# pengpeng-yu/FastPCC

Measured on AMD Instinct MI355X. Metric: encode+decode Mpoints/sec, lossy_coord_v2 baseline_r1 (stream of 16-frame batches, 2 in flight; one frame at a time = value_one_frame), higher is better.
Workload: dtype f32; 1 GPU; lossy_coord_v2/baseline_r1 inference, 997645-voxel 1024^3 body-surface frames (cfg#2), seeded random-init weights; one step = a batch of 16 such frames per GPU (15966320 voxels) through compress_many + decompress_many = ONE network traversal over the batch, 16 independent streams; 2 batch(es) in flight per GPU; parallelism=single GPU, 2 batches in flight per GPU on one stream (fastpcc_amd/serving.py), batch_clouds=16, frames_in_flight=2, named_stages=False, bytes=143901, coder_handover_retries=0

## Files before the change

fastpcc_amd/codecs/lossy_coord_v2/layers.py:

```python
from typing import List, Optional, Tuple

import torch
import torch.nn as nn
import torch.nn.functional as F

from ... import engine as ME
from ... import hipops as ops
from ...sparse_conv_layers import ConvBlock, ConvTransBlock, GenConvTransBlock, MEMLPBlock, \
    NNSequentialWithConvBlockArgs, NNSequentialWithConvTransBlockArgs, mlp_chain_forward


def _run(seq: nn.Sequential, x, last_clip: float = 0.0):
    mods = list(seq)
    for m in mods[:-1]:
        x = m(x)
    return mods[-1](x, clip=last_clip) if last_clip > 0 else mods[-1](x)


def classify_head(seq: nn.Sequential, fea):
    blocks = list(seq)
    ok = len(blocks) == 2 and not torch.is_grad_enabled() and len(fea.parts) == 1
    if ok:
        a, b = blocks
        ok = all(isinstance(m, ConvBlock) and m.bn is None and m.conv.ks == 1 and
                 (m.act_module is None or isinstance(m.act_module, (ME.MinkowskiPReLU, ME.MinkowskiReLU))) for m in blocks) and \
            b.conv.out_channels == 1 and a.conv.out_channels == b.conv.in_channels and \
            ops.pointwise_head_ok(a.conv.in_channels, a.conv.out_channels)
    x = fea.parts[0] if ok else None
    if not ok or x.dtype != torch.float32 or x.stride(1) != 1 or (x.shape[0] > 1 and x.stride(0) % 4) or x.data_ptr() % 16:
        return seq(fea)
    da, db = a.conv._derived(), b.conv._derived()
    act1, act2 = ME._act_of(a.act_module), ME._act_of(b.act_module)
    cm = fea.coordinate_manager
    orders = {ME.summation_order('k1', a.conv.in_channels, 0, a.conv.out_channels, rows)
              for rows in cm.cloud_rows(cm._map(fea.coordinate_map_key)) if rows > 0}
    if len(orders) != 1 or not orders <= {0, 1}:
        return seq(fea)
    order1 = orders.pop()
    out = ops.pointwise_head(x, da['w'].reshape(a.conv.in_channels, a.conv.out_channels), da['b'], act1.kind, act1.slope, order1,
                             db['w'].reshape(-1), db['b'], act2.kind, act2.slope)
    return ME.SparseTensor(out, coordinate_map_key=fea.coordinate_map_key, coordinate_manager=fea.coordinate_manager)


class Encoder(nn.Module):

    def __init__(self, in_channels: int, intra_channels: Tuple[int, ...], requires_points_num_list: bool,
                 points_num_scaler: float, region_type: str, act: Optional[str]):
        super().__init__()
        self.requires_points_num_list = requires_points_num_list
        self.points_num_scaler = points_num_scaler
        stages = [ConvBlock(in_channels, intra_channels[0], 3, 1, region_type=region_type, act=act)]
        for c_prev, c in zip(intra_channels[:-1], intra_channels[1:]):
            stages.append(nn.Sequential(
                ConvBlock(c_prev, c, 2, 2, region_type='HYPER_CUBE', act=act),
                ConvBlock(c, c, 3, 1, region_type=region_type, act=act)))
        self.blocks = nn.ModuleList(stages)

    def forward(self, x) -> Tuple[ME.SparseTensor, Optional[List[List[int]]]]:
        counts = []
        last = len(self.blocks) - 1
        for i, block in enumerate(self.blocks):
            x = block(x)
            if i != last:
                cm = x.coordinate_manager
                edges = cm.batch_offsets(cm._map(x.coordinate_map_key))
                counts.append([b - a for a, b in zip(edges[:-1], edges[1:])])
        if not self.requires_points_num_list:
            return x, None
        return x, [[int(n * self.points_num_scaler) for n in c] for c in counts]


class Decoder(nn.Module):

    def __init__(self, in_channels: int, intra_channels: Tuple[int, ...], region_type: str, act: Optional[str]):
        super().__init__()
        self.upsample_blocks = nn.ModuleList()
        self.classify_blocks = nn.ModuleList()
        prev = in_channels
        n_stage = len(intra_channels)
        for i, ch in enumerate(intra_channels):
            up = nn.Sequential()
            if i == n_stage - 1:
                up.append(ConvBlock(prev, prev, 3, 1, region_type=region_type, act=act))
            up.append(GenConvTransBlock(prev, ch, 2, 2, region_type='HYPER_CUBE', act=act))
            if i != n_stage - 1:
                up.append(ConvBlock(ch, ch, 3, 1, region_type=region_type, act=act))
            self.upsample_blocks.append(up)
            self.classify_blocks.append(nn.Sequential(ConvBlock(ch, ch // 2, 1, 1, act=act),
                                                      ConvBlock(ch // 2, 1, 1, 1, act=None)))
            prev = ch
        self.pruning = ME.MinkowskiPruning()

    def forward(self, fea, points_num_list, coord_offset=None):
        if self.training:
            return self.train_forward(fea, points_num_list, coord_offset)
        return self.test_forward(fea, points_num_list, coord_offset)

    def train_forward(self, fea, points_num_list, target_key: ME.CoordinateMapKey) -> dict:
        loss = {}
        n_stage = len(self.upsample_blocks)
        cm = fea.coordinate_manager
        top = cm._map(fea.coordinate_map_key)
        inv = [1 / sum(c) for c in points_num_list] if points_num_list is not None else None
        for i, (up, classify) in enumerate(zip(self.upsample_blocks, self.classify_blocks)):
            fea = up(fea)
            pred = classify(fea)
            keep = self.get_keep_train(pred, points_num_list, top)
            target = self.get_target(pred, target_key)
            keep |= target
            loss[f'coord_{n_stage - i - 1}_recon_loss'] = F.binary_cross_entropy_with_logits(
                pred.F.squeeze(1), target.to(pred.F.dtype), reduction='sum')
            if i != n_stage - 1:
                fea = self.pruning(fea, keep.to(torch.uint8))
        if inv is not None and len(inv) != 1:
            total = sum(inv)
            for i in range(n_stage):
                loss[f'coord_{i}_recon_loss'] = loss[f'coord_{i}_recon_loss'] * (inv[i] / total * len(inv))
        return loss

    @torch.no_grad()
    def get_target(self, pred: ME.SparseTensor, target_key: ME.CoordinateMapKey) -> torch.Tensor:
        cm = pred.coordinate_manager
        gen = cm._map(pred.coordinate_map_key)
        tgt = cm._map(cm.stride(target_key, pred.tensor_stride))
        if gen.generated and tgt.parent is gen.parent:
            self.last_target_path = 'child_table'
            return ops.child_mask(tgt.child_row).bool()
        if gen.level != tgt.level or gen.bits != tgt.bits:
            raise ValueError('candidates and strided target set differ in tensor stride')
        self.last_target_path = 'keys_member'
        return ops.keys_member(cm._keys(tgt), cm._keys(gen)) >= 0

    @torch.no_grad()
    def get_keep_train(self, pred: ME.SparseTensor, points_num_list: Optional[List[List[int]]], top) -> torch.Tensor:
        cm = pred.coordinate_manager
        gen = cm._map(pred.coordinate_map_key)
        if not gen.generated:
            raise NotImplementedError('get_keep expects the candidates of a generative upsampling')
        parent = gen.parent
        logits = pred.F.detach().reshape(-1).contiguous()
        cell = None
        if parent is not top:
            cell = cm._ancestor_rows(parent, top).to(torch.int32).contiguous()
        if points_num_list is None:
            return fixed_keep(logits, cell, 0 if cell is None else top.n).bool()
        targets = points_num_list.pop()
        edges = cm.batch_offsets(parent)
        if len(targets) != len(edges) - 1:
            raise ValueError('one pruning target per sample expected')
        return ops.topk_keep_batch(logits, edges, targets, cell, 0 if cell is None else top.n).bool()

    @torch.no_grad()
    def test_forward(self, fea, points_num_list, coord_offset: Optional[torch.Tensor] = None):
        last = len(self.upsample_blocks) - 1
        cm = fea.coordinate_manager
        top = cm._map(fea.coordinate_map_key)
        for i, (up, classify) in enumerate(zip(self.upsample_blocks, self.classify_blocks)):
            fea = up(fea)
            keep = self.get_keep(classify_head(classify, fea), points_num_list, top)
            if i != last:
                fea = self.pruning(fea, keep)
            else:
                gen = cm._map(fea.coordinate_map_key)
                if not gen.generated:
                    raise RuntimeError('decoder output is expected on a generated coordinate set')
                if not cm.independent_clouds:
                    xyz, count = ops.compact_coords(gen.parent.keys, keep, gen.level, gen.bits, coord_offset)
                    return xyz[:int(count.item())]
                edges = cm.batch_offsets(gen.parent)
                parts = [ops.compact_coords(gen.parent.keys[a:b], keep[8 * a: 8 * b], gen.level, gen.bits,
                                            None if coord_offset is None else coord_offset[c].contiguous())
                         for c, (a, b) in enumerate(zip(edges[:-1], edges[1:]))]
                counts = torch.cat([count for _, count in parts]).tolist()
                return [xyz[:n] for (xyz, _), n in zip(parts, counts)]

    @torch.no_grad()
    def get_keep(self, pred: ME.SparseTensor, points_num_list: Optional[List[List[int]]], top=None) -> torch.Tensor:
        cm = pred.coordinate_manager
        gen = cm._map(pred.coordinate_map_key)
        if not gen.generated:
            raise NotImplementedError('get_keep expects the candidates of a generative upsampling')
        logits = pred.F.view(-1)
        parent = gen.parent
        cell = None
        if top is not None and parent is not top:
            cell, m = parent.parent_of, parent.parent
            while m is not top:
                if m is None or m.parent_of is None:
                    raise RuntimeError('candidate set is not below the decoder input level')
                cell, m = m.parent_of[cell.long()], m.parent
            cell = cell.to(torch.int32).contiguous()
        if points_num_list is None:
            return fixed_keep(logits, cell, 0 if cell is None else top.n)
        return adaptive_keep(cm, parent, top, logits, cell, points_num_list.pop())


def fixed_keep(logits: torch.Tensor, cell: Optional[torch.Tensor], n_cells: int) -> torch.Tensor:
    groups = logits.view(-1, 8)
    per_group = groups.max(1).values
    if cell is None:
        return ((groups > 0) | (groups == per_group[:, None])).view(-1).to(torch.uint8)
    cell_max = torch.full((n_cells,), float('-inf'), dtype=per_group.dtype, device=per_group.device)
    cell_max.scatter_reduce_(0, cell.long(), per_group, reduce='amax', include_self=True)
    return ((groups > 0) | (groups == cell_max[cell.long()][:, None])).view(-1).to(torch.uint8)


def adaptive_keep(cm, parent, top, logits: torch.Tensor, cell: Optional[torch.Tensor], target: List[int]) -> torch.Tensor:
    if cm.independent_clouds:
        edges = cm.batch_offsets(parent)
        if len(target) != len(edges) - 1:
            raise ValueError('one pruning target per cloud expected')
        return ops.topk_keep_batch(logits, edges, target, cell, 0 if cell is None else top.n)
    if len(target) != 1:
        raise NotImplementedError('batch size 1 at test time, as in the reference (model.py:121)')
    if not logits.numel() > target[0]:
        raise ValueError('fewer candidates than points to keep')
    if cell is None:
        return ops.topk_keep(logits, target[0])
    return ops.topk_keep_cells(logits, cell, top.n, target[0])


class HyperDecoderUpsample(nn.Module):

    def __init__(self, in_channels: Tuple[int, ...], out_channels: Tuple[int, ...], if_sample: Tuple[int, ...],
                 region_type: str, act: Optional[str]):
        super().__init__()
        self.blocks = nn.ModuleList()
        for c_in, c_out, up in zip(in_channels, out_channels, if_sample):
            if up:
                head = ConvTransBlock(max(c_in, 1), c_out, 2, 2, region_type=region_type, act=act)
                seq = NNSequentialWithConvTransBlockArgs
            else:
                head = ConvBlock(max(c_in, 1), c_out, 3, 1, region_type=region_type, act=act)
                seq = NNSequentialWithConvBlockArgs
            self.blocks.append(seq(head, ConvBlock(c_out, c_out, 3, 1, region_type=region_type, act=act)))

    def __len__(self):
        return len(self.blocks)

    def __getitem__(self, idx):
        return self.blocks[idx]


class HyperDecoderGenUpsample(nn.Module):

    def __init__(self, in_channels: Tuple[int, ...], if_sample: Tuple[int, ...], region_type: str, act: Optional[str]):
        super().__init__()
        self.blocks = nn.ModuleList()
        for c_in, up in zip(in_channels, if_sample):
            if not up:
                self.blocks.append(None)
                continue
            mid = max(c_in // 4, 1)
            self.blocks.append(nn.Sequential(
                GenConvTransBlock(c_in, mid, 2, 2, region_type=region_type, act=act),
                ConvBlock(mid, 1, 3, 1, region_type=region_type, act=None)))

    def __getitem__(self, idx):
        return self.blocks[idx]


class SubResidualGeoLossl(nn.Module):

    def __init__(self, in_ch, out_ch, region_type, act, bottleneck_value_bound: int):
        super().__init__()
        self.blocks = nn.Sequential(
            ConvBlock(in_ch + in_ch, in_ch, 3, 1, region_type=region_type, act=act),
            ConvBlock(in_ch, out_ch, 3, 1, region_type=region_type, act=None))
        self.register_buffer('bound', torch.tensor(bottleneck_value_bound), persistent=False)
        self._bound = float(bottleneck_value_bound)

    def forward(self, x, y):
        return _run(self.blocks, ME.cat(x, y), last_clip=self._bound)


class ResidualGeoLossl(nn.Module):
    def __init__(self, in_channels: Tuple[int, ...], out_channels: Tuple[int, ...], region_type: str,
                 act: Optional[str], bottleneck_value_bound: int, skip_encoding_fea: int):
        super().__init__()
        self.blocks = nn.ModuleList()
        for idx, (c_in, c_out) in enumerate(zip(in_channels, out_channels)):
            self.blocks.append(SubResidualGeoLossl(c_in, c_out, region_type, act, bottleneck_value_bound)
                               if idx > skip_encoding_fea else None)

    def __len__(self):
        return len(self.blocks)

    def __getitem__(self, idx):
        return self.blocks[idx]


class SubDecoderGeoLossl(nn.Module):

    def __init__(self, in_ch, in_ch2, out_ch, region_type, act):
        super().__init__()
        self.residual_decoder = nn.Sequential(MEMLPBlock(in_ch, out_ch // 2, act=act),
                                              MEMLPBlock(out_ch // 2, out_ch, act=act))
        self.decoder = nn.Sequential(MEMLPBlock(out_ch + in_ch2, out_ch, act=act),
                                     MEMLPBlock(out_ch, out_ch, act=act))

    def forward(self, x, y: ME.SparseTensor):
        fused = mlp_chain_forward([*self.residual_decoder, *self.decoder], x, y, cat_layer=len(self.residual_decoder))
        if fused is not None:
            return ME.SparseTensor(fused, coordinate_map_key=y.coordinate_map_key, coordinate_manager=y.coordinate_manager)
        if isinstance(x, torch.Tensor):
            x = ME.SparseTensor(x, coordinate_map_key=y.coordinate_map_key, coordinate_manager=y.coordinate_manager)
        return self.decoder(ME.cat(self.residual_decoder(x), y))


class SubDecoderGeoLossl2(nn.Module):
    def __init__(self, in_ch, in_ch2, out_ch, region_type, act):
        super().__init__()
# ... 63 lines not shown
```

fastpcc_amd/csrc/hip/conv.hip:

```cpp
#include "conv_common.h"
#include <atomic>
#include <cstdlib>

namespace fpcc {
namespace {

template <int NBT, int CH, int WM, int WN>
struct MfmaCfg {
    static constexpr int C_OUT = 32 * NBT;
    static constexpr int TM = 32 * WM;
    static constexpr int NBW = NBT / WN;
    static constexpr int THREADS = 64 * WM * WN;
    static constexpr int G8 = CH / 8;
    static constexpr int W_TOTAL = CH * C_OUT / 4;
    static constexpr int W_PIECES = (W_TOTAL + THREADS - 1) / THREADS;
    static_assert(NBT % WN == 0, "column blocks must divide over the waves");
};

template <typename C, int CH>
__device__ __forceinline__ void fetch_a(const ConvArgs &a, const int32_t *nbr_rows, int cc, int li, int lh,
                                        f32x4 (&ra)[C::G8]) {
    const bool in_x1 = cc * CH < a.c1;
    const float *xb = in_x1 ? a.x1 + cc * CH : a.x2 + (cc * CH - a.c1);
    const int64_t ld = in_x1 ? a.ld1 : a.ld2;
// ... 813 lines not shown
        const float *ap[2], *bp;
        auto next_stage = [&]() {
            const bool in1 = cc_f < n1;
            const int c = in1 ? cc_f : cc_f - n1;
            ap[0] = (in1 ? a1[0] : a2[0]) + c * step[0];
            ap[1] = (in1 ? a1[1] : a2[1]) + c * step[1];
            bp = bpk + cc_f * chunk_floats;
            if (cc_f + 1 < n_chunks) {
                ++cc_f;
            } else {
                const unsigned r2 = rest & (rest - 1);
                if (r2) { rest = r2; cc_f = 0; set_offset(__ffs(r2) - 1); }
            }
        };
        f32x4 ra[2][G8], rbv[G8][2];
        next_stage();
#pragma unroll
        for (int g8 = 0; g8 < G8; ++g8) {
            __builtin_amdgcn_sched_barrier(0);
            ra[0][g8] = *reinterpret_cast<const f32x4 *>(ap[0] + 8 * g8);
            __builtin_amdgcn_sched_barrier(0);
            ra[1][g8] = *reinterpret_cast<const f32x4 *>(ap[1] + 8 * g8);
#pragma unroll
            for (int nb = 0; nb < 2; ++nb) {
                __builtin_amdgcn_sched_barrier(0);
                rbv[g8][nb] = *reinterpret_cast<const f32x4 *>(bp + ((int64_t)g8 * nbt + nb) * 256);
            }
        }
        __builtin_amdgcn_sched_barrier(0);
        for (int s = 0; s < n_stages; ++s) {
            if (cc_c == 0) {
                const int gk = offset_group_of(__ffs(rest_c) - 1, n_off);
                if (gk != cur_g) {
                    fold_acc();
                    for (int gz = cur_g + 1; gz < gk; ++gz) fold_zero();
                    cur_g = gk;
                }
            }
            if (++cc_c == n_chunks) { cc_c = 0; rest_c &= rest_c - 1; }
            next_stage();
            __builtin_amdgcn_sched_barrier(SB);
#pragma unroll
            for (int g8 = 0; g8 < G8; ++g8) {
                const f32x4 av0 = ra[0][g8], av1 = ra[1][g8];
                const f32x4 b0 = rbv[g8][0], b1 = rbv[g8][1];
#define FPCC_STEP(c)                                                                                     \
                acc[0][0] = __builtin_amdgcn_mfma_f32_32x32x2f32(av0.c, b0.c, acc[0][0], 0, 0, 0);       \
                acc[0][1] = __builtin_amdgcn_mfma_f32_32x32x2f32(av0.c, b1.c, acc[0][1], 0, 0, 0);       \
                acc[1][0] = __builtin_amdgcn_mfma_f32_32x32x2f32(av1.c, b0.c, acc[1][0], 0, 0, 0);       \
                acc[1][1] = __builtin_amdgcn_mfma_f32_32x32x2f32(av1.c, b1.c, acc[1][1], 0, 0, 0);
                FPCC_STEP(x) FPCC_STEP(y) FPCC_STEP(z) FPCC_STEP(w)
#undef FPCC_STEP
                __builtin_amdgcn_sched_barrier(SB);
                ra[0][g8] = *reinterpret_cast<const f32x4 *>(ap[0] + 8 * g8);
                __builtin_amdgcn_sched_barrier(SB);
                ra[1][g8] = *reinterpret_cast<const f32x4 *>(ap[1] + 8 * g8);
#pragma unroll
                for (int nb = 0; nb < 2; ++nb) {
                    __builtin_amdgcn_sched_barrier(SB);
                    rbv[g8][nb] = *reinterpret_cast<const f32x4 *>(bp + ((int64_t)g8 * nbt + nb) * 256);
                }
                __builtin_amdgcn_sched_barrier(SB);
            }
        }
    }
    if (wmask) { fold_acc(); ++cur_g; }
    for (int gz = cur_g; gz < 4; ++gz) fold_zero();

    const float slope = (a.act == FPCC_ACT_PRELU && a.slope) ? a.slope[0] : 0.0f;
    float bias2[2];
#pragma unroll
    for (int nb = 0; nb < 2; ++nb) bias2[nb] = a.bias ? a.bias[32 * ((int)cg * 2 + nb) + li] : 0.0f;
#pragma unroll
    for (int rb = 0; rb < 2; ++rb) {
        int64_t dsts[16];
#pragma unroll
        for (int reg = 0; reg < 16; ++reg) {
            const int64_t o = __shfl(my_row, 32 * rb + (reg & 3) + 8 * (reg >> 2) + 4 * lh);
            dsts[reg] = o < 0 ? -1 : o;
        }
#pragma unroll
        for (int reg = 0; reg < 16; ++reg) {
            const int64_t dst = dsts[reg];
            if (dst < 0) continue;
#pragma unroll
            for (int nb = 0; nb < 2; ++nb)
                a.out[dst * a.ldo + 32 * ((int)cg * 2 + nb) + li] = finish(tsum[rb][nb][reg], bias2[nb], a.act, slope, a.clip);
        }
    }
}

__global__ __launch_bounds__(256) void k_pack_weights(const float *__restrict__ w, int64_t n_mats, int c_in, int c_out,
                                                      float *__restrict__ wp) {
    const int64_t e = (int64_t)blockIdx.x * 256 + threadIdx.x;
    const int64_t per_mat = (int64_t)c_in * c_out;
    if (e >= n_mats * per_mat) return;
    const int nbt = c_out / 32;
    const int64_t m = e / per_mat;
    int64_t r = e - m * per_mat;
    const int j = (int)(r & 3); r >>= 2;
    const int i = (int)(r & 31); r >>= 5;
    const int h = (int)(r & 1); r >>= 1;
    const int nb = (int)(r % nbt); r /= nbt;
    const int g8 = (int)(r & 3); r >>= 2;
    const int cc = (int)r;
    wp[e] = w[m * per_mat + (int64_t)(32 * cc + 8 * g8 + 4 * h + j) * c_out + 32 * nb + i];
}

__global__ __launch_bounds__(256) void k_pack_weights_nat(const float *__restrict__ w, int64_t n_mats, int c_in, int c_out,
                                                          float *__restrict__ wp) {
    const int64_t e = (int64_t)blockIdx.x * 256 + threadIdx.x;
    const int64_t per_mat = (int64_t)c_in * c_out;
    if (e >= n_mats * per_mat) return;
    const int nbt = c_out / 32;
    const int64_t m = e / per_mat;
    int64_t r = e - m * per_mat;
    const int j = (int)(r & 3); r >>= 2;
    const int i = (int)(r & 31); r >>= 5;
    const int h = (int)(r & 1); r >>= 1;
    const int nb = (int)(r % nbt); r /= nbt;
    const int g8 = (int)(r & 3); r >>= 2;
    const int cc = (int)r;
    wp[e] = w[m * per_mat + (int64_t)(32 * cc + 8 * g8 + 2 * j + h) * c_out + 32 * nb + i];
}

inline bool aligned16(const void *p) { return (reinterpret_cast<uintptr_t>(p) & 15) == 0; }

int mfma_chunk(int c1, int c2, int c_out) {
    if (c_out != 32 && c_out != 64 && c_out != 128) return 0;
    const int c_in = c1 + c2;
    if (c_in % 32 == 0 && c1 % 32 == 0) return 32;
    if (c_in % 16 == 0 && c1 % 16 == 0) return 16;
    return 0;
}

bool natural_shape(int c1, int c2, int c_out, int n_offsets, int groups) {
    return c_out == 256 && c1 >= 32 && c1 % 32 == 0 && c2 >= 0 && c2 % 32 == 0 && c1 + c2 <= 512 && n_offsets >= 1 && n_offsets <= kMaxOffsets &&
           (groups == 1 || groups == 8);
}

int knob(int k);

template <int NBT, int CH, int WM, int WN>
int launch_mfma_cfg(ConvArgs a, hipStream_t s) {
    constexpr int TM = 32 * WM;
    const unsigned tiles = (unsigned)((a.n_out + TM - 1) / TM);
    const dim3 grid(tiles, a.groups), block(64 * WM * WN);
    hipLaunchKernelGGL((k_conv_mfma<NBT, CH, WM, WN>), grid, block, 0, s, a);
    return check_hip(hipGetLastError(), "k_conv_mfma");
}

enum { kKnobWaveOn = 0, kKnobWaveNbw = 1, kKnobWaveSb = 2, kKnobStamps = 3, kKnobGroupedFoldRows = 4, kKnobMfmaCfg = 5, kKnobPointwiseRows = 6,
       kKnobGroupedOff = 7, kKnobGroupedNbw = 8, kKnobWave22Rows = 9, kKnobLdsRows = 10, kKnobLdsRowBlocks = 11, kKnobPersist = 12, kKnobFold64 = 13, kKnobK2s2tSparse = 14,
       kKnobNaturalMfma = 15, kKnobCount = 16 };
int g_knob[kKnobCount] = {-1, -1, -1, -1, -1, -1, -1, -1, -1, -1, -1, -1, -1, -1, -1, -1};
int knob(int k) {
    if (g_knob[k] < 0) {
        static const char *names[kKnobCount] = {"FPCC_CONV_WAVE", "FPCC_WAVE_NBW", "FPCC_WAVE_SB", "", "FPCC_GROUPED_FOLD_ROWS",
                                                "FPCC_MFMA_TILE", "FPCC_POINTWISE_MIN_ROWS", "", "FPCC_GROUPED_NBW",
                                                "FPCC_WAVE22_MIN_ROWS", "FPCC_LDS_MIN_ROWS", "FPCC_LDS_ROW_BLOCKS",
                                                "FPCC_CONV_PERSIST", "FPCC_CONV_FOLD64", "FPCC_K2S2T_SPARSE",
                                                "FPCC_CONV_NATURAL_MFMA"};
        static const int defaults[kKnobCount] = {1, 0, 1, 0, 100 * 1024, 0, 32 * 1024, 0, 0, 0, 0, 2, 0, 0, 0, 2};
        const char *e = names[k][0] ? getenv(names[k]) : nullptr;
        g_knob[k] = e ? atoi(e) : defaults[k];
    }
    return g_knob[k];
}

template <int NBT, int CH>
int launch_mfma(const ConvArgs &a, hipStream_t s) {
    const int forced = knob(kKnobMfmaCfg) - 1;
    const int64_t work = a.n_out * a.groups;
    constexpr int WNS = NBT >= 2 ? 2 : 1;
    const int cfg = forced >= 0 ? forced : (NBT <= 2 && work >= 128 * 1024) ? 0 : work >= 32 * 1024 ? 1 : 2;
    if (cfg == 0) return launch_mfma_cfg<NBT, CH, 4, 1>(a, s);
    if (cfg == 1) return launch_mfma_cfg<NBT, CH, 2, WNS>(a, s);
    return launch_mfma_cfg<NBT, CH, 1, NBT>(a, s);
}

__global__ __launch_bounds__(256) void k_conv_c1_pointwise(ConvArgs a) {
    const int64_t e = (int64_t)blockIdx.x * 256 + threadIdx.x;
    if (e >= a.n_out * a.c_out) return;
    const int64_t o = e / a.c_out;
    const int j = (int)(e - o * a.c_out);
    const float slope = (a.act == FPCC_ACT_PRELU && a.slope) ? a.slope[0] : 0.0f;
    a.out[o * a.ldo + j] = finish(fmaf(a.x1[o * a.ld1], a.w[j], 0.0f), a.bias ? a.bias[j] : 0.0f, a.act, slope, a.clip);
}

template <int NBW>
int launch_wave_cfg(const ConvArgs &a, const float *wp, int nbt, hipStream_t s) {
    const int64_t row_blocks = (a.n_out + 31) / 32;
    const int64_t units = row_blocks * (nbt / NBW);
    if (units > 0x7fffffffll) return fail_arg("conv_f32: too many work units");
    const dim3 grid((unsigned)((units + 3) / 4), a.groups);
    if (knob(kKnobWaveSb)) hipLaunchKernelGGL((k_conv_wave<NBW, 32, 0x6>), grid, dim3(256), 0, s, a, wp, nbt, (unsigned)units);
    else hipLaunchKernelGGL((k_conv_wave<NBW, 32, 0>), grid, dim3(256), 0, s, a, wp, nbt, (unsigned)units);
    return check_hip(hipGetLastError(), "k_conv_wave");
}

constexpr int kMaxDevices = 16;
inline int current_device() {
    int dev = 0;
    return (hipGetDevice(&dev) == hipSuccess && dev >= 0 && dev < kMaxDevices) ? dev : -1;
}
int cu_count() {
    static std::atomic<int> cached[kMaxDevices];
    const int dev = current_device();
    if (dev < 0) return 256;
    int n = cached[dev].load(std::memory_order_relaxed);
    if (n == 0) {
        hipDeviceProp_t prop;
        n = (hipGetDeviceProperties(&prop, dev) == hipSuccess && prop.multiProcessorCount > 0) ? prop.multiProcessorCount : 256;
        cached[dev].store(n, std::memory_order_relaxed);
    }
    return n;
}

constexpr int kUnitCounters = 256;
__device__ unsigned g_unit_counters[kUnitCounters];
unsigned *next_unit_counter(unsigned start, hipStream_t s, int *rc) {
    static std::atomic<unsigned> seq{0};
    static std::atomic<unsigned *> bases[kMaxDevices];
    const int dev = current_device();
    if (dev < 0) {
        *rc = fail_arg("unit counters: no current device");
        return nullptr;
    }
    unsigned *base = bases[dev].load(std::memory_order_acquire);
    if (!base) {
        if (hipGetSymbolAddress(reinterpret_cast<void **>(&base), HIP_SYMBOL(g_unit_counters)) != hipSuccess) {
            *rc = check_hip(hipGetLastError(), "unit counters");
            return nullptr;
        }
        bases[dev].store(base, std::memory_order_release);
    }
    unsigned *c = base + (seq++ % kUnitCounters);
    *rc = check_hip(hipMemsetD32Async(reinterpret_cast<hipDeviceptr_t>(c), (int)start, 1, s), "unit counter fill");
    return c;
}

inline int64_t persist_slots() {
    const int v = knob(kKnobPersist);
    return v > 16 ? v : (int64_t)v * cu_count();
}
inline bool persist_ok(const ConvArgs &a) {
    return knob(kKnobPersist) > 0 && a.nbr && a.nbr_ks == 1 && (a.nbr_os & 3) == 0 && a.nbr_os >= ((a.n_off + 3) & ~3) &&
           (reinterpret_cast<uintptr_t>(a.nbr) & 15) == 0 && a.groups == 1;
}

template <int NBW>
int launch_grouped_cfg(const ConvArgs &a, const float *wp, int nbt, hipStream_t s) {
    const int64_t row_blocks = (a.n_out + 31) / 32;
    const int64_t units = row_blocks * (nbt / NBW);
    if (units > 0x7fffffffll) return fail_arg("conv_f32: too many work units");
    const bool stamps = knob(kKnobStamps) != 0;
    const int64_t slots = persist_slots();
    if (!stamps && persist_ok(a) && units > slots) {
        int rc = FPCC_OK;
        unsigned *counter = next_unit_counter((unsigned)slots, s, &rc);
        if (rc != FPCC_OK) return rc;
        hipLaunchKernelGGL((k_conv_wave<NBW, 32, 0x6, false, 4, false, true>), dim3((unsigned)slots, 1), dim3(256), 0, s, a, wp, nbt, (unsigned)units,
                           counter);
        return check_hip(hipGetLastError(), "k_conv_wave(grouped, persistent)");
    }
    if (stamps)
        hipLaunchKernelGGL((k_conv_wave<NBW, 32, 0x6, true, 4>), dim3((unsigned)units, a.groups), dim3(256), 0, s, a, wp, nbt, (unsigned)units);
    else
        hipLaunchKernelGGL((k_conv_wave<NBW, 32, 0x6, false, 4>), dim3((unsigned)units, a.groups), dim3(256), 0, s, a, wp, nbt, (unsigned)units);
    return check_hip(hipGetLastError(), "k_conv_wave(grouped)");
}

template <int NBW>
int launch_folded_cfg(const ConvArgs &a, const float *wp, int nbt, hipStream_t s) {
    const int64_t units = ((a.n_out + 31) / 32) * (nbt / NBW);
    if (units > 0x7fffffffll) return fail_arg("conv_f32: too many work units");
    const int64_t slots = persist_slots();
    if (!knob(kKnobStamps) && persist_ok(a) && (units + 3) / 4 > slots) {
        int rc = FPCC_OK;
        unsigned *counter = next_unit_counter((unsigned)(4 * slots), s, &rc);
        if (rc != FPCC_OK) return rc;
        hipLaunchKernelGGL((k_conv_wave<NBW, 32, 0x6, false, 1, true, true>), dim3((unsigned)slots, 1), dim3(256), 0, s, a, wp, nbt, (unsigned)units,
                           counter);
        return check_hip(hipGetLastError(), "k_conv_wave(folded, persistent)");
    }
    hipLaunchKernelGGL((k_conv_wave<NBW, 32, 0x6, false, 1, true>), dim3((unsigned)((units + 3) / 4), a.groups), dim3(256), 0, s, a, wp, nbt,
                       (unsigned)units);
    return check_hip(hipGetLastError(), "k_conv_wave(folded)");
}

constexpr int64_t kFold64Rows = 200 * 1024;
std::atomic<long long> g_fold64_launches{0};
inline bool use_fold64(const ConvArgs &a, int nbt) {
    if ((nbt != 2 && nbt != 4) || (a.n_off != kMaxOffsets && a.n_off != 8) || knob(kKnobPersist) > 0) return false;
    const int v = knob(kKnobFold64);
    if (v) return v >= 2;
    return a.row_order && a.n_out >= kFold64Rows;
}

int launch_fold64(const ConvArgs &a, const float *wp, int nbt, hipStream_t s) {
    const int64_t units = ((a.n_out + 63) / 64) * (nbt / 2);
    if (units > 0x7fffffffll) return fail_arg("conv_f32: too many work units");
    hipLaunchKernelGGL(k_conv_fold64, dim3((unsigned)((units + 3) / 4), 1), dim3(256), 0, s, a, wp, nbt, (unsigned)units);
    g_fold64_launches.fetch_add(1, std::memory_order_relaxed);
    return check_hip(hipGetLastError(), "k_conv_fold64");
}

int launch_grouped(const ConvArgs &a, const float *wp, hipStream_t s) {
    const int nbt = a.c_out / 32;
    const int64_t lds_rows = knob(kKnobLdsRows);
    if (lds_rows > 0 && a.n_out >= lds_rows) {
        const int rc = launch_conv_lds(a, wp, knob(kKnobLdsRowBlocks), knob(kKnobStamps) != 0, s);
        if (rc != -1) return rc;
    }
    const int64_t fold_rows = knob(kKnobGroupedFoldRows);
    if (fold_rows > 0 && a.n_out >= fold_rows && knob(kKnobGroupedNbw) <= 0) {
        if (use_fold64(a, nbt)) return launch_fold64(a, wp, nbt, s);
        return nbt % 2 == 0 ? launch_folded_cfg<2>(a, wp, nbt, s) : launch_folded_cfg<1>(a, wp, nbt, s);
    }
    int nbw = knob(kKnobGroupedNbw);
    if (nbw <= 0) nbw = a.n_out >= 40 * 1024 ? 2 : 1;
    while (nbw > nbt || nbt % nbw) nbw >>= 1;
    return nbw == 2 ? launch_grouped_cfg<2>(a, wp, nbt, s) : launch_grouped_cfg<1>(a, wp, nbt, s);
}

int launch_wave22(const ConvArgs &a, const float *wp, int nbt, hipStream_t s) {
    const int64_t units = ((a.n_out + 63) / 64) * (nbt / 2);
    if (units > 0x7fffffffll) return fail_arg("conv_f32: too many work units");
    const dim3 grid((unsigned)((units + 3) / 4), a.groups);
    if (knob(kKnobWaveSb)) hipLaunchKernelGGL((k_conv_wave22<0x6>), grid, dim3(256), 0, s, a, wp, nbt, (unsigned)units);
    else hipLaunchKernelGGL((k_conv_wave22<0>), grid, dim3(256), 0, s, a, wp, nbt, (unsigned)units);
    return check_hip(hipGetLastError(), "k_conv_wave22");
}

int launch_wave(const ConvArgs &a, const float *wp, hipStream_t s) {
    const int nbt = a.c_out / 32;
    const int64_t work = a.n_out * a.groups;
    const int64_t rows22 = knob(kKnobWave22Rows);
    if (rows22 > 0 && a.n_off > 1 && nbt % 2 == 0 && work >= rows22 && knob(kKnobWaveNbw) <= 0) return launch_wave22(a, wp, nbt, s);
    int nbw = knob(kKnobWaveNbw);
    if (nbw <= 0) nbw = work >= 32 * 1024 ? 2 : 1;
    while (nbw > nbt || nbt % nbw) nbw >>= 1;
    if (nbw >= 4) return launch_wave_cfg<4>(a, wp, nbt, s);
    if (nbw == 2) return launch_wave_cfg<2>(a, wp, nbt, s);
    return launch_wave_cfg<1>(a, wp, nbt, s);
}


constexpr int64_t kNaturalMfmaRows = 0;
std::atomic<long long> g_natural_launches{0};
inline bool use_natural_mfma(int64_t work) {
    const int v = knob(kKnobNaturalMfma);
    return v == 1 || (v >= 2 && work >= kNaturalMfmaRows);
}

template <int NBW>
int launch_natural_cfg(const ConvArgs &a, const float *wp, hipStream_t s) {
    constexpr int nbt = 8;
    const int64_t units = ((a.n_out + 31) / 32) * (nbt / NBW);
    if (units > 0x7fffffffll) return fail_arg("conv_f32: too many work units");
    hipLaunchKernelGGL((k_conv_wave<NBW, 32, 0x6, false, 1, false, false, true>), dim3((unsigned)((units + 3) / 4), a.groups), dim3(256), 0, s, a,
                       wp, nbt, (unsigned)units);
    g_natural_launches.fetch_add(1, std::memory_order_relaxed);
    return check_hip(hipGetLastError(), "k_conv_wave(natural)");
}

int launch_natural(const ConvArgs &a, const float *wp, hipStream_t s) {
    int nbw = knob(kKnobWaveNbw);
    if (nbw <= 0) nbw = a.n_out * a.groups >= 32 * 1024 ? 2 : 1;
    return nbw >= 2 ? launch_natural_cfg<2>(a, wp, s) : launch_natural_cfg<1>(a, wp, s);
}

template <int NBW, int NCH>
__global__ __launch_bounds__(256, 2) void k_pointwise_wave(ConvArgs a, const float *__restrict__ wp, int nbt, unsigned n_row_blocks,
                                                           unsigned waves_per_cg) {
    constexpr int AC = NCH < 4 ? NCH : 4;
    constexpr int TW = 32 * NBW + 4;
    __shared__ float s_tile[4][32 * TW];
    const int lane = threadIdx.x & 63, wv = threadIdx.x >> 6;
    const int li = lane & 31, lh = lane >> 5;
    const unsigned n_cg = (unsigned)(nbt / NBW);
    const unsigned w = blockIdx.x * 4u + (unsigned)wv;
    const unsigned cg = w % n_cg, slot = w / n_cg;
    if (slot >= waves_per_cg) return;

    f32x4 rb[NCH][4][NBW];
    {
        const float *wpl = wp + ((int64_t)cg * NBW) * 256 + lane * 4;
#pragma unroll
        for (int cc = 0; cc < NCH; ++cc)
#pragma unroll
            for (int g8 = 0; g8 < 4; ++g8)
#pragma unroll
                for (int nb = 0; nb < NBW; ++nb)
                    rb[cc][g8][nb] = *reinterpret_cast<const f32x4 *>(wpl + (((int64_t)cc * 4 + g8) * nbt + nb) * 256);
    }
    const int n1 = a.c1 / 32;
    const float slope = (a.act == FPCC_ACT_PRELU && a.slope) ? a.slope[0] : 0.0f;
    float bias[NBW];
#pragma unroll
    for (int nb = 0; nb < NBW; ++nb) bias[nb] = a.bias ? a.bias[32 * ((int)cg * NBW + nb) + li] : 0.0f;

    auto row_ptrs = [&](unsigned rbk, const float *&q1, const float *&q2) {
        int64_t row = (int64_t)rbk * 32 + li;
        if (row >= a.n_out) row = a.n_out - 1;
        q1 = a.x1 + row * a.ld1 + 4 * lh;
        q2 = a.x2 ? a.x2 + row * a.ld2 + 4 * lh : q1;
    };
    auto fetch = [&](const float *q1, const float *q2, int cc, int g8) -> f32x4 {
        const float *src = cc < n1 ? q1 + 32 * cc : q2 + 32 * (cc - n1);
        return *reinterpret_cast<const f32x4 *>(src + 8 * g8);
    };
    const float *c1p, *c2p, *n1p, *n2p;
    row_ptrs(slot, c1p, c2p);
    f32x4 ra[AC][4];
#pragma unroll
    for (int c = 0; c < AC; ++c)
#pragma unroll
        for (int g8 = 0; g8 < 4; ++g8) {
            __builtin_amdgcn_sched_barrier(0);
            ra[c][g8] = fetch(c1p, c2p, c, g8);
        }
    __builtin_amdgcn_sched_barrier(0);
    for (unsigned rbk = slot; rbk < n_row_blocks; rbk += waves_per_cg) {
        const int64_t row0 = (int64_t)rbk * 32;
        row_ptrs(rbk + waves_per_cg, n1p, n2p);
        f32x16 acc[NBW];
#pragma unroll
        for (int nb = 0; nb < NBW; ++nb)
#pragma unroll
            for (int r = 0; r < 16; ++r) acc[nb][r] = 0.0f;
#pragma unroll
        for (int cc = 0; cc < NCH; ++cc) {
            constexpr int kNone = 0;
            (void)kNone;
            const int sl = cc % AC;
            const bool wraps = cc + AC >= NCH;
            const int cn = (cc + AC) % NCH;
#pragma unroll
            for (int g8 = 0; g8 < 4; ++g8) {
                const f32x4 av = ra[sl][g8];
#pragma unroll
                for (int nb = 0; nb < NBW; ++nb) acc[nb] = __builtin_amdgcn_mfma_f32_32x32x2f32(av.x, rb[cc][g8][nb].x, acc[nb], 0, 0, 0);
#pragma unroll
                for (int nb = 0; nb < NBW; ++nb) acc[nb] = __builtin_amdgcn_mfma_f32_32x32x2f32(av.y, rb[cc][g8][nb].y, acc[nb], 0, 0, 0);
#pragma unroll
                for (int nb = 0; nb < NBW; ++nb) acc[nb] = __builtin_amdgcn_mfma_f32_32x32x2f32(av.z, rb[cc][g8][nb].z, acc[nb], 0, 0, 0);
#pragma unroll
                for (int nb = 0; nb < NBW; ++nb) acc[nb] = __builtin_amdgcn_mfma_f32_32x32x2f32(av.w, rb[cc][g8][nb].w, acc[nb], 0, 0, 0);
                __builtin_amdgcn_sched_barrier(0x6);
                ra[sl][g8] = wraps ? fetch(n1p, n2p, cn, g8) : fetch(c1p, c2p, cn, g8);
                __builtin_amdgcn_sched_barrier(0x6);
            }
        }
        c1p = n1p;
        c2p = n2p;
        float *tile = s_tile[wv];
#pragma unroll
        for (int reg = 0; reg < 16; ++reg) {
            const int r = (reg & 3) + 8 * (reg >> 2) + 4 * lh;
#pragma unroll
            for (int nb = 0; nb < NBW; ++nb) tile[r * TW + 32 * nb + li] = finish(acc[nb][reg], bias[nb], a.act, slope, a.clip);
        }
        __builtin_amdgcn_wave_barrier();
        constexpr int LPR = 8 * NBW;
        constexpr int RPI = 64 / LPR;
        const int qr = lane / LPR, qc = lane % LPR;
#pragma unroll
        for (int r0 = 0; r0 < 32; r0 += RPI) {
            const int r = r0 + qr;
            const f32x4 v = *reinterpret_cast<const f32x4 *>(tile + r * TW + 4 * qc);
            const int64_t o = row0 + r;
            if (o < a.n_out)
                *reinterpret_cast<f32x4 *>(a.out + o * a.ldo + 32 * (int)cg * NBW + 4 * qc) = v;
        }
        __builtin_amdgcn_wave_barrier();
    }
}


template <int NBW, int NCH>
int launch_pointwise_cfg(const ConvArgs &a, const float *wp, int nbt, hipStream_t s) {
    const unsigned row_blocks = (unsigned)((a.n_out + 31) / 32);
    const unsigned n_cg = (unsigned)(nbt / NBW);
    unsigned waves_per_cg = (256u * 4u * 2u) / n_cg;
    if (waves_per_cg > row_blocks) waves_per_cg = row_blocks;
    const unsigned waves = waves_per_cg * n_cg;
    hipLaunchKernelGGL((k_pointwise_wave<NBW, NCH>), dim3((waves + 3) / 4), dim3(256), 0, s, a, wp, nbt, row_blocks, waves_per_cg);
    return check_hip(hipGetLastError(), "k_pointwise_wave");
}

int launch_pointwise(const ConvArgs &a, const float *wp, hipStream_t s) {
    const int nbt = a.c_out / 32, nch = (a.c1 + a.c2) / 32;
    switch (nch) {
        case 1: return nbt % 4 == 0 ? launch_pointwise_cfg<4, 1>(a, wp, nbt, s) : nbt % 2 == 0 ? launch_pointwise_cfg<2, 1>(a, wp, nbt, s)
                                                                                                : launch_pointwise_cfg<1, 1>(a, wp, nbt, s);
        case 2: return nbt % 4 == 0 ? launch_pointwise_cfg<4, 2>(a, wp, nbt, s) : nbt % 2 == 0 ? launch_pointwise_cfg<2, 2>(a, wp, nbt, s)
                                                                                                : launch_pointwise_cfg<1, 2>(a, wp, nbt, s);
        case 4: return nbt % 2 == 0 ? launch_pointwise_cfg<2, 4>(a, wp, nbt, s) : launch_pointwise_cfg<1, 4>(a, wp, nbt, s);
        case 8: return launch_pointwise_cfg<1, 8>(a, wp, nbt, s);
        default: return -1;
    }
}


typedef float f32x2_t __attribute__((ext_vector_type(2)));
template <int CO, int R>
__global__ __launch_bounds__(256) void k_conv_ones_k3(const uint32_t *__restrict__ masks, int64_t n, const float *__restrict__ w,
                                                      const float *__restrict__ bias, int act, const float *__restrict__ slope, float clip,
                                                      float *__restrict__ out, int ldo) {
    const int64_t base = (int64_t)blockIdx.x * (256 * R) + threadIdx.x;
    uint32_t m[R];
#pragma unroll
    for (int i = 0; i < R; ++i) { const int64_t r = base + i * 256; m[i] = r < n ? masks[r] : 0u; }
    f32x2_t acc[R][CO / 2];
#pragma unroll
    for (int i = 0; i < R; ++i)
#pragma unroll
        for (int p = 0; p < CO / 2; ++p) acc[i][p] = {0.0f, 0.0f};
    f32x2_t wcur[CO / 2];
#pragma unroll
    for (int p = 0; p < CO / 2; ++p) wcur[p] = {w[2 * p], w[2 * p + 1]};
#pragma unroll 1
    for (int k = 0; k < 27; ++k) {
        const float *wn = w + (k < 26 ? k + 1 : 26) * CO;
        f32x2_t wnext[CO / 2];
#pragma unroll
        for (int p = 0; p < CO / 2; ++p) wnext[p] = {wn[2 * p], wn[2 * p + 1]};
        f32x2_t bb[R];
#pragma unroll
        for (int i = 0; i < R; ++i) {
            const float bit = __int_as_float((((int32_t)(m[i] << (31 - k))) >> 31) & 0x3f800000);
            bb[i] = {bit, bit};
        }
#pragma unroll
        for (int p = 0; p < CO / 2; ++p)
#pragma unroll
            for (int i = 0; i < R; ++i) acc[i][p] = __builtin_elementwise_fma(bb[i], wcur[p], acc[i][p]);
#pragma unroll
        for (int p = 0; p < CO / 2; ++p) wcur[p] = wnext[p];
    }
    const float sl = (act == FPCC_ACT_PRELU && slope) ? slope[0] : 0.0f;
    static_assert(R == 1, "one row per thread");
    __shared__ float s_rows[256 * (CO + 1)];
    float *mine = s_rows + threadIdx.x * (CO + 1);
#pragma unroll
    for (int h = 0; h < CO / 4; ++h) {
        mine[4 * h] = finish(acc[0][2 * h].x, bias ? bias[4 * h] : 0.0f, act, sl, clip);
        mine[4 * h + 1] = finish(acc[0][2 * h].y, bias ? bias[4 * h + 1] : 0.0f, act, sl, clip);
        mine[4 * h + 2] = finish(acc[0][2 * h + 1].x, bias ? bias[4 * h + 2] : 0.0f, act, sl, clip);
        mine[4 * h + 3] = finish(acc[0][2 * h + 1].y, bias ? bias[4 * h + 3] : 0.0f, act, sl, clip);
    }
    __syncthreads();
    const int64_t row0 = (int64_t)blockIdx.x * 256;
    constexpr int kPieces = CO / 4;
#pragma unroll
    for (int j = 0; j < kPieces; ++j) {
        const int e = j * 256 + (int)threadIdx.x;
        const int r = e / kPieces, piece = e - r * kPieces;
        if (row0 + r < n) {
            const float *src = s_rows + r * (CO + 1) + 4 * piece;
            f32x4 o;
            o.x = src[0]; o.y = src[1]; o.z = src[2]; o.w = src[3];
            *reinterpret_cast<f32x4 *>(out + (row0 + r) * ldo + 4 * piece) = o;
        }
    }
}

template <int CO>
int launch_ones_k3(const uint32_t *masks, int64_t n, const float *w, const float *bias, int act, const float *slope, float clip,
                   float *out, int ldo, hipStream_t s) {
    hipLaunchKernelGGL((k_conv_ones_k3<CO, 1>), dim3(blocks_for(n, 256)), dim3(256), 0, s, masks, n, w, bias, act, slope, clip, out, ldo);
    return check_hip(hipGetLastError(), "k_conv_ones_k3");
}

template <int JB>
int launch_valu(const ConvArgs &a, hipStream_t s) {
    const int n_jb = (a.c_out + JB - 1) / JB;
    hipLaunchKernelGGL((k_conv_valu<JB>), dim3(blocks_for(a.n_out, 256), a.groups * n_jb), dim3(256), 0, s, a, n_jb);
    return check_hip(hipGetLastError(), "k_conv_valu");
}

}
}

using namespace fpcc;

static fpcc_conv_plan conv_plan(int c1, int c2, int c_out, int n_offsets, int groups) {
    fpcc_conv_plan p{};
    p.chunk = mfma_chunk(c1, c2, c_out);
    const bool nat = natural_shape(c1, c2, c_out, n_offsets, groups);
    const bool wave = p.chunk == 32 && n_offsets >= 1 && n_offsets <= kMaxOffsets && groups >= 1;
    const bool grouped = wave && n_offsets >= 8 && groups == 1 && !knob(kKnobGroupedOff);
    p.order = grouped ? 3 : p.chunk ? 1 : 0;
    p.matrix = p.chunk || nat;
    p.packed = nat ? 2 : wave ? 1 : 0;
    p.packed_floats = p.packed ? (int64_t)groups * n_offsets * (c1 + c2) * c_out : 0;
    p.ws_bytes = grouped || nat ? 4 * p.packed_floats : 0;
    return p;
}

extern "C" int fpcc_conv_f32_plan(int c1, int c2, int c_out, int n_offsets, int groups, fpcc_conv_plan *plan) {
    if (!plan) return fail_arg("conv_f32_plan: null pointer");
    *plan = conv_plan(c1, c2, c_out, n_offsets, groups);
    return FPCC_OK;
}

extern "C" int fpcc_conv_f32_order(int c1, int c2, int c_out) { return conv_plan(c1, c2, c_out, 1, 1).order; }
extern "C" int fpcc_conv_f32_order_ex(int c1, int c2, int c_out, int n_offsets, int groups, int64_t) {
    return conv_plan(c1, c2, c_out, n_offsets, groups).order;
}
extern "C" int fpcc_conv_f32_natural_matrix(int c1, int c2, int c_out, int n_offsets, int groups) {
    return conv_plan(c1, c2, c_out, n_offsets, groups).packed == 2;
}
extern "C" int64_t fpcc_conv_f32_ws_bytes(int c1, int c2, int c_out, int n_offsets, int groups, int64_t n_out) {
    return n_out > 0 ? conv_plan(c1, c2, c_out, n_offsets, groups).ws_bytes : 0;
}
static int64_t packed_floats_of(const fpcc_conv_plan &p, int image) { return p.packed == image ? p.packed_floats : 0; }
extern "C" int64_t fpcc_conv_packed_floats(int c1, int c2, int c_out, int n_offsets, int groups) {
    return packed_floats_of(conv_plan(c1, c2, c_out, n_offsets, groups), 1);
}
extern "C" int64_t fpcc_conv_packed_floats_nat(int c1, int c2, int c_out, int n_offsets, int groups) {
    return packed_floats_of(conv_plan(c1, c2, c_out, n_offsets, groups), 2);
}

extern "C" int fpcc_conv_natural_use_matrix(int64_t rows) { return use_natural_mfma(rows) ? 1 : 0; }

extern "C" long long fpcc_conv_natural_launches(void) { return g_natural_launches.load(std::memory_order_relaxed); }

extern "C" int fpcc_numerics_version(void) { return FPCC_NUMERICS_VERSION; }

extern "C" int fpcc_conv_ones_k3_f32(const uint32_t *masks, int64_t n, const float *w, const float *bias, int c_out, int act,
                                     const float *slope, float clip, float *out, int ldo, void *stream) {
    if (n < 0 || c_out < 4 || c_out > 32 || c_out % 4 || ldo < c_out || ldo % 4) return fail_arg("conv_ones_k3: 4 <= c_out <= 32, multiple of 4");
    if (n == 0) return FPCC_OK;
    if (!masks || !w || !out || !aligned16(out)) return fail_arg("conv_ones_k3: null or unaligned pointer");
    if (act == FPCC_ACT_PRELU && !slope) return fail_arg("conv_ones_k3: PReLU needs a slope pointer");
    hipStream_t st = as_stream(stream);
    switch (c_out) {
        case 4: return launch_ones_k3<4>(masks, n, w, bias, act, slope, clip, out, ldo, st);
        case 8: return launch_ones_k3<8>(masks, n, w, bias, act, slope, clip, out, ldo, st);
        case 12: return launch_ones_k3<12>(masks, n, w, bias, act, slope, clip, out, ldo, st);
        case 16: return launch_ones_k3<16>(masks, n, w, bias, act, slope, clip, out, ldo, st);
        case 20: return launch_ones_k3<20>(masks, n, w, bias, act, slope, clip, out, ldo, st);
        case 24: return launch_ones_k3<24>(masks, n, w, bias, act, slope, clip, out, ldo, st);
        case 28: return launch_ones_k3<28>(masks, n, w, bias, act, slope, clip, out, ldo, st);
        default: return launch_ones_k3<32>(masks, n, w, bias, act, slope, clip, out, ldo, st);
    }
}

extern "C" int fpcc_conv_debug_stamps(unsigned long long *buf, int64_t n_u64) {
    if (n_u64 < 0 || (n_u64 > 0 && !buf)) return fail_arg("conv_debug_stamps: null buffer");
    const long long cap = buf ? n_u64 : 0;
    FPCC_HIP(hipMemcpyToSymbol(HIP_SYMBOL(g_stamp_buf), &buf, sizeof(buf)));
    FPCC_HIP(hipMemcpyToSymbol(HIP_SYMBOL(g_stamp_cap), &cap, sizeof(cap)));
    return set_lds_stamp_buffer(buf, cap);
}

extern "C" long long fpcc_conv_fold64_launches(void) { return g_fold64_launches.load(std::memory_order_relaxed); }

extern "C" int fpcc_conv_set_tuning(int which, int value) {
    if (which < 0 || which >= kKnobCount) return fail_arg("conv_set_tuning: unknown knob");
    if (which == kKnobGroupedOff) {
        const char *e = getenv("FPCC_EXPERIMENT");
        if (!e || atoi(e) != 1)
            return fail_arg("conv_set_tuning: the summation order is part of the stream format (FPCC_EXPERIMENT=1 to override)");
    }
    if (which == kKnobStamps && value != 0 && value != 16)
        return fail_arg("conv_set_tuning: knob 3 is 0 or 16 (stamped builds); the timing ablations are no longer part of the library");
    const int before = knob(which);
    g_knob[which] = value < 0 ? 0 : value;
    return before;
}

extern "C" int fpcc_conv_pack_weights_nat_f32(const float *w, int64_t n_mats, int c_in, int c_out, float *w_packed, void *stream) {
    if (n_mats < 0 || c_in < 32 || c_in % 32 || c_in > 512 || c_out != 256)
        return fail_arg("conv_pack_weights_nat: c_in must be a multiple of 32 (<= 512) and c_out 256");
    if (n_mats == 0) return FPCC_OK;
    if (!w || !w_packed) return fail_arg("conv_pack_weights_nat: null pointer");
    hipLaunchKernelGGL(k_pack_weights_nat, dim3(blocks_for(n_mats * c_in * c_out, 256)), dim3(256), 0, as_stream(stream), w, n_mats,
                       c_in, c_out, w_packed);
    return check_hip(hipGetLastError(), "k_pack_weights_nat");
}

extern "C" int fpcc_conv_pack_weights_f32(const float *w, int64_t n_mats, int c_in, int c_out, float *w_packed, void *stream) {
    if (n_mats < 0 || c_in < 32 || c_in % 32 || (c_out != 32 && c_out != 64 && c_out != 128))
        return fail_arg("conv_pack_weights: c_in must be a multiple of 32 and c_out one of 32, 64, 128");
    if (n_mats == 0) return FPCC_OK;
    if (!w || !w_packed) return fail_arg("conv_pack_weights: null pointer");
    hipLaunchKernelGGL(k_pack_weights, dim3(blocks_for(n_mats * c_in * c_out, 256)), dim3(256), 0, as_stream(stream), w, n_mats,
                       c_in, c_out, w_packed);
    return check_hip(hipGetLastError(), "k_pack_weights");
}

extern "C" int fpcc_conv_f32(const float *x1, int c1, int ld1, const float *x2, int c2, int ld2, const int32_t *nbr,
                             int n_offsets, int64_t nbr_ks, int64_t nbr_os, const float *w, const float *bias, int c_out,
                             int groups, const int32_t *out_map, int64_t om_os, int64_t om_gs, float *out, int ldo,
                             int64_t n_out, int act, const float *slope, float clip, const int32_t *row_order,
                             void *ws, int64_t ws_bytes, void *stream) {
    return fpcc_conv_f32_pk(x1, c1, ld1, x2, c2, ld2, nbr, n_offsets, nbr_ks, nbr_os, w, nullptr, bias, c_out, groups, out_map,
                            om_os, om_gs, out, ldo, n_out, act, slope, clip, row_order, ws, ws_bytes, stream);
}

namespace fpcc {
PendingEvents &pending_events() {
    static thread_local PendingEvents p;
    return p;
}
}

extern "C" int fpcc_time_next_launch(void *start_event, void *end_event) {
    PendingEvents &p = pending_events();
    p.ev0 = start_event;
    p.ev1 = end_event;
    return FPCC_OK;
}

extern "C" int fpcc_conv_f32_pk(const float *x1, int c1, int ld1, const float *x2, int c2, int ld2, const int32_t *nbr,
                                int n_offsets, int64_t nbr_ks, int64_t nbr_os, const float *w, const float *w_packed,
                                const float *bias, int c_out, int groups, const int32_t *out_map, int64_t om_os,
                                int64_t om_gs, float *out, int ldo, int64_t n_out, int act, const float *slope, float clip,
                                const int32_t *row_order, void *ws, int64_t ws_bytes, void *stream) {
    LaunchBracket timed(stream);
    if (n_out < 0 || c1 < 1 || c2 < 0 || c_out < 1 || groups < 1 || n_offsets < 1 || n_offsets > 32)
        return fail_arg("conv_f32: sizes out of range (n_offsets must be 1..32)");
    if (n_out == 0) return FPCC_OK;
    if (!x1 || !w || !out || (c2 > 0 && !x2)) return fail_arg("conv_f32: null pointer");
    if (!nbr && n_offsets != 1) return fail_arg("conv_f32: identity map needs n_offsets == 1");
    if (ld1 < c1 || (c2 > 0 && ld2 < c2) || ldo < c_out) return fail_arg("conv_f32: row stride smaller than the row");
    if (act != FPCC_ACT_NONE && act != FPCC_ACT_PRELU && act != FPCC_ACT_RELU) return fail_arg("conv_f32: unknown activation");
    if (act == FPCC_ACT_PRELU && !slope) return fail_arg("conv_f32: PReLU needs a slope pointer");
    if ((int64_t)groups * ((c_out + 15) / 16) > 65535) return fail_arg("conv_f32: too many groups");

    ConvArgs a{x1, c1, ld1, x2, c2, ld2, nbr, n_offsets, nbr_ks, nbr_os, w, bias, c_out, groups,
               out_map, om_os, om_gs, out, ldo, n_out, act, slope, clip, row_order};
    hipStream_t s = as_stream(stream);
    const fpcc_conv_plan plan = conv_plan(c1, c2, c_out, n_offsets, groups);
    const int ch = plan.chunk;
    if (row_order && !plan.matrix)
        return fail_arg("conv_f32: row_order is a feature of the matrix path (fpcc_conv_f32_order() != 0 or fpcc_conv_f32_natural_matrix())");
    const bool nat_operands = aligned16(x1) && ld1 % 4 == 0 && (c2 == 0 || (aligned16(x2) && ld2 % 4 == 0)) &&
                              (w_packed ? aligned16(w_packed) : (ws && aligned16(ws) && ws_bytes >= plan.ws_bytes));
    if (plan.packed == 2 && nat_operands && use_natural_mfma(n_out * (int64_t)groups)) {
        const float *wp = w_packed;
        if (!wp) {
            if (int rc = fpcc_conv_pack_weights_nat_f32(w, (int64_t)groups * n_offsets, c1 + c2, c_out, static_cast<float *>(ws), stream)) return rc;
            wp = static_cast<const float *>(ws);
        }
        return launch_natural(a, wp, s);
    }
    if (ch && n_offsets > kMaxOffsets) return fail_arg("conv_f32: the MFMA path supports at most 27 kernel offsets");
    if (ch && !(aligned16(x1) && ld1 % 4 == 0 && aligned16(w) && (c2 == 0 || (aligned16(x2) && ld2 % 4 == 0))))
        return fail_arg("conv_f32: the MFMA path needs 16-byte aligned inputs and row strides that are multiples of 4");
    if (nbr && plan.order == 3) {
        if (out_map) return fail_arg("conv_f32: grouped shapes do not take an output map");
        const float *wp = w_packed;
        if (!wp) {
            if (!ws || ws_bytes < plan.ws_bytes || !aligned16(ws))
                return fail_arg("conv_f32: this shape needs packed weights or a 16-byte aligned workspace of fpcc_conv_f32_ws_bytes() bytes");
            if (int rc = fpcc_conv_pack_weights_f32(w, n_offsets, c1 + c2, c_out, static_cast<float *>(ws), stream)) return rc;
            wp = static_cast<const float *>(ws);
        } else if (!aligned16(wp)) {
            return fail_arg("conv_f32: packed weights must be 16-byte aligned");
        }
        return launch_grouped(a, wp, s);
    }
    if (ch == 16 && c2 == 0 && c1 == 48 && c_out <= 64 && n_out * (int64_t)groups >= 32 * 1024)
        return c_out == 64 ? launch_mfma_cfg<2, 48, 4, 1>(a, s) : launch_mfma_cfg<1, 48, 4, 1>(a, s);
    if (ch == 32 && w_packed) {
        if (!aligned16(w_packed)) return fail_arg("conv_f32: packed weights must be 16-byte aligned");
        if (knob(kKnobWaveOn)) {
            const int64_t pw_rows = knob(kKnobPointwiseRows);
            if (n_offsets == 1 && !nbr && !row_order && groups == 1 && !out_map && pw_rows > 0 && n_out >= pw_rows && aligned16(out) &&
                ldo % 4 == 0) {
                const int rc = launch_pointwise(a, w_packed, s);
                if (rc != -1) return rc;
            }
            return launch_wave(a, w_packed, s);
        }
    }
    if (ch == 32) {
        if (c_out == 128) return launch_mfma<4, 32>(a, s);
        if (c_out == 64) return launch_mfma<2, 32>(a, s);
        return launch_mfma<1, 32>(a, s);
    }
    if (ch == 16) {
        if (c_out == 128) return launch_mfma<4, 16>(a, s);
        if (c_out == 64) return launch_mfma<2, 16>(a, s);
        return launch_mfma<1, 16>(a, s);
    }
    if (c1 == 1 && c2 == 0 && n_offsets == 1 && !nbr && groups == 1 && !out_map && c_out >= 8) {
        hipLaunchKernelGGL(k_conv_c1_pointwise, dim3(blocks_for(n_out * c_out, 256)), dim3(256), 0, s, a);
        return check_hip(hipGetLastError(), "k_conv_c1_pointwise");
    }
    if (c_out == 1) return launch_valu<1>(a, s);
    if (c_out <= 4) return launch_valu<4>(a, s);
    if (c_out <= 8) return launch_valu<8>(a, s);
    return launch_valu<16>(a, s);
}

namespace fpcc {
namespace {
__global__ void k_conv_row_keys(const int32_t *__restrict__ nbr, int n_off, int64_t nbr_ks, int64_t nbr_os, int64_t n,
// ... 419 lines not shown
```

fastpcc_amd/engine.py:

```python
import functools
import math
import os
from enum import Enum
from typing import Dict, List, Optional, Sequence, Tuple, Union

import torch
import torch.nn as nn

from . import hipops as ops
from .autograd import conv_autocast


class RegionType(Enum):
    HYPER_CUBE = 0
    HYPER_CROSS = 1
    CUSTOM = 2


class MinkowskiAlgorithm(Enum):
    DEFAULT = 0
    MEMORY_EFFICIENT = 1
    SPEED_OPTIMIZED = 2


# ... 363 lines not shown
        if ks == 2 and st == 2:
            if a.parent is not b or a.generated:
                raise NotImplementedError('kernel_map(kernel_size=2, stride=2) maps a level onto its stride-2 parent')
            out = {}
            for k in range(8):
                rows_out = torch.nonzero(a.child_row[:, k] >= 0).squeeze(1)
                if rows_out.numel():
                    out[k] = torch.stack((a.child_row[rows_out, k].long(), rows_out))
            return out
        if ks != 1:
            raise NotImplementedError(f'kernel_map(kernel_size={ks}, stride={st})')
        if a.level != b.level:
            raise NotImplementedError('kernel_map(kernel_size=1) needs maps of equal stride')
        ka, kb = self._keys(a), self._keys(b)
        if kb.numel() == 0 or ka.numel() == 0:
            return {}
        pos = torch.searchsorted(kb, ka).clamp_(max=kb.numel() - 1)
        hit = kb[pos] == ka
        rows_in = torch.nonzero(hit).squeeze(1)
        return {0: torch.stack((rows_in, pos[hit]))}

    def origin_map(self, key: CoordinateMapKey):
        m = self._map(key)
        edges = self.batch_offsets(m)
        dev = self.device if m.keys is None else m.keys.device
        return CoordinateMapKey(1, 'origin'), [torch.arange(a, b, device=dev) for a, b in zip(edges[:-1], edges[1:])]

    def _ancestor_rows(self, m: _Map, target: _Map) -> torch.Tensor:
        if m is target:
            raise ValueError('the maps are the same')
        dev = self.device if m.keys is None and m.parent.keys is None else (m.keys if m.keys is not None else m.parent.keys).device
        idx = torch.arange(m.n, device=dev)
        cur = m
        while cur is not target:
            if cur.parent is None:
                raise ValueError('the target map is not an ancestor of the input map')
            idx = torch.div(idx, 8, rounding_mode='floor') if cur.generated else cur.parent_of.long()[idx]
            cur = cur.parent
        return idx

    def batch_offsets(self, m: _Map) -> List[int]:
        if m.edges is not None:
            return m.edges
        if m.n == 0:
            return [0]
        if self._n_batch == 1:
            m.edges = [0, m.n]
        elif m.generated and m.parent is not None and m.parent.n * 8 == m.n:
            m.edges = [8 * e for e in self.batch_offsets(m.parent)]
        else:
            b = (self._keys(m) >> (3 * m.bits))
            nb = self._n_batch if self.independent_clouds else int(b[-1].item()) + 1
            m.edges = torch.searchsorted(b, torch.arange(nb + 1, device=b.device, dtype=b.dtype)).tolist()
        return m.edges

    def cloud_rows(self, m: _Map) -> List[int]:
        if not self.independent_clouds:
            return [m.n]
        e = self.batch_offsets(m)
        return [b - a for a, b in zip(e[:-1], e[1:])]


def _edges_of(counts: Sequence[int]) -> List[int]:
    edges = [0]
    for c in counts:
        edges.append(edges[-1] + int(c))
    return edges


class SparseTensor:

    def __init__(self, features: Union[torch.Tensor, Tuple[torch.Tensor, torch.Tensor]], coordinates=None,
                 tensor_stride=1, coordinate_map_key: Optional[CoordinateMapKey] = None,
                 coordinate_manager: Optional[CoordinateManager] = None,
                 quantization_mode: SparseTensorQuantizationMode = SparseTensorQuantizationMode.RANDOM_SUBSAMPLE,
                 **_):
        if coordinate_manager is None:
            coordinate_manager = global_coordinate_manager() \
                if _operation_mode == SparseTensorOperationMode.SHARE_COORDINATE_MANAGER else None
            if coordinate_manager is None:
                coordinate_manager = CoordinateManager()
                if _operation_mode == SparseTensorOperationMode.SHARE_COORDINATE_MANAGER:
                    set_global_coordinate_manager(coordinate_manager)
        self.coordinate_manager = coordinate_manager
        if coordinates is not None:
            if coordinate_map_key is not None:
                raise ValueError('give coordinates or a coordinate_map_key, not both')
            key, (rows, n) = coordinate_manager.insert_and_map(coordinates, tensor_stride)
            if n != coordinates.shape[0] and quantization_mode == SparseTensorQuantizationMode.UNWEIGHTED_AVERAGE:
                features = _average_duplicates(features, coordinate_manager, key, coordinates, tensor_stride)
            else:
                features = ops.gather_rows(features.contiguous(), rows.contiguous())
            coordinate_map_key = key
        elif coordinate_map_key is None:
            raise ValueError('coordinates or coordinate_map_key required')
        self.coordinate_map_key = coordinate_map_key
        self._parts = features if isinstance(features, tuple) else (features,)
        n_rows = coordinate_manager._map(coordinate_map_key).n
        for f in self._parts:
            if f.shape[0] != n_rows:
                raise ValueError(f'features have {f.shape[0]} rows, the coordinate map {n_rows}')

    @property
    def F(self) -> torch.Tensor:
        if len(self._parts) > 1:
            self._parts = (torch.cat(self._parts, dim=1),)
        return self._parts[0]

    @property
    def parts(self) -> Tuple[torch.Tensor, ...]:
        return self._parts

    @property
    def C(self) -> torch.Tensor:
        return self.coordinate_manager.get_coordinates(self.coordinate_map_key)

    @property
    def tensor_stride(self) -> List[int]:
        return self.coordinate_map_key.get_tensor_stride()

    @property
    def shape(self):
        return torch.Size((self._parts[0].shape[0], sum(p.shape[1] for p in self._parts)))

    @property
    def device(self):
        return self._parts[0].device

    @property
    def dtype(self):
        return self._parts[0].dtype

    def size(self):
        return self.shape

    @property
    def _batchwise_row_indices(self):
        edges = self.coordinate_manager.batch_offsets(self.coordinate_manager._map(self.coordinate_map_key))
        return [torch.arange(a, b, device=self.device) for a, b in zip(edges[:-1], edges[1:])]

    @property
    def decomposition_permutations(self):
        return self._batchwise_row_indices

    @property
    def decomposed_coordinates(self):
        c = self.C
        return [c[idx, 1:] for idx in self._batchwise_row_indices]

    def __repr__(self):
        return f'SparseTensor(shape={tuple(self.shape)}, key={self.coordinate_map_key})'


def _average_duplicates(features, cm, key, coordinates, tensor_stride):
    m = cm._map(key)
    level = m.level
    keys = ops.keys_from_coords(coordinates.contiguous(), level, m.bits)
    row = torch.searchsorted(m.keys, keys)
    out = torch.zeros((m.n, features.shape[1]), dtype=features.dtype, device=features.device)
    cnt = torch.zeros((m.n, 1), dtype=features.dtype, device=features.device)
    out.index_add_(0, row, features)
    cnt.index_add_(0, row, torch.ones_like(features[:, :1]))
    return out / cnt


def cat(*tensors) -> SparseTensor:
    if len(tensors) == 1 and isinstance(tensors[0], (tuple, list)):
        tensors = tuple(tensors[0])
    key, cm = tensors[0].coordinate_map_key, tensors[0].coordinate_manager
    parts = []
    for t in tensors:
        if t.coordinate_manager is not cm or cm._map(t.coordinate_map_key) is not cm._map(key):
            raise ValueError('cat needs tensors on the same coordinate map')
        parts.extend(t.parts)
    if len(parts) > 2:
        parts = [torch.cat(parts[:-1], dim=1), parts[-1]]
    return SparseTensor(tuple(parts), coordinate_map_key=key, coordinate_manager=cm)


class _Act:
    __slots__ = ('kind', 'slope', 'param')

    def __init__(self, kind=ops.ACT_NONE, slope=None, param=None):
        self.kind, self.slope, self.param = kind, slope, param


def _act_of(module: Optional[nn.Module]) -> _Act:
    if module is None:
        return _Act()
    if isinstance(module, MinkowskiPReLU):
        w = module.module.weight
        cached = module.__dict__.get('_fpcc_act')
        if cached is None or cached[0] != w.data_ptr():
            if w.numel() != 1:
                raise NotImplementedError('per-channel PReLU')
            cached = (w.data_ptr(), _Act(ops.ACT_PRELU, w.detach(), w))
            module.__dict__['_fpcc_act'] = cached
        return cached[1]
    if isinstance(module, MinkowskiReLU):
        return _Act(ops.ACT_RELU)
    raise NotImplementedError(f'cannot fuse {type(module).__name__}')


def _packed_gen_ok(c_in: int, c_out: int) -> bool:
    return c_in % 16 == 0 and 8 * c_out in (32, 64, 128, 256)


def _split_k3_ok(c_in: int, c2: int, c_out: int) -> bool:
    return c_out == 1 and c2 == 0 and c_in % 16 == 0


PAD_MIN_ROWS = 8192


@functools.lru_cache(maxsize=4096)
def _pad_plan(c1: int, c2: int, c_out: int, n_out: int):
    if ops.conv_order(c1, c2, c_out) != 0 or c_out > 128 or c1 + c2 < 4 or (c1 + c2) * c_out < 32 or n_out < PAD_MIN_ROWS:
        return None
    c1p = (c1 + 15) // 16 * 16
    c2p = (c2 + 15) // 16 * 16 if c2 else 0
    c_outp = 32 if c_out <= 32 else (64 if c_out <= 64 else 128)
    return c1p, c2p, c_outp


def _layer_form(kind: str, c1: int, c2: int, c_out: int, rows: int):
    if kind == 'gen' and c2 == 0 and _packed_gen_ok(c1, c_out):
        return 'gen', (c1, c2, c_out)
    if kind == 'k3' and _split_k3_ok(c1, c2, c_out):
        return 'split', (c1, c2, c_out)
    plan = _pad_plan(c1, c2, c_out, rows) if kind in ('k1', 'k3') else None
    return ('plain', (c1, c2, c_out)) if plan is None else ('pad', plan)


def summation_order(kind: str, c1: int, c2: int, c_out: int, n_out: int = 0) -> int:
    form, shape = _layer_form(kind, c1, c2, c_out, n_out)
    if form in ('gen', 'split'):
        return 1 if form == 'gen' else 2
    return ops.conv_order(*shape, {'k3': 27, 'k2s2': 8}.get(kind, 1), 8 if kind in ('gen', 'k2s2T') else 1)


class _ConvBase(nn.Module):
    TRANSPOSED = False
    GENERATIVE = False

    def __init__(self, in_channels, out_channels, kernel_size=-1, stride=1, dilation=1, bias=False,
                 kernel_generator: Optional[KernelGenerator] = None, expand_coordinates=False, dimension=3):
        super().__init__()
        if kernel_generator is None:
            kernel_generator = KernelGenerator(kernel_size, stride, dilation, dimension=dimension)
        kg = kernel_generator
        if len(set(kg.kernel_size)) != 1 or len(set(kg.kernel_stride)) != 1 or set(kg.kernel_dilation) != {1}:
            raise NotImplementedError('isotropic kernels without dilation only')
        self.kernel_generator = kg
        self.in_channels, self.out_channels = in_channels, out_channels
        self.ks, self.st = kg.kernel_size[0], kg.kernel_stride[0]
        if (self.ks, self.st) not in ((1, 1), (3, 1), (2, 2)):
            raise NotImplementedError(f'kernel {self.ks} stride {self.st}')
        if (self.TRANSPOSED or self.GENERATIVE) and (self.ks, self.st) != (2, 2):
            raise NotImplementedError('transposed convolutions are kernel 2 stride 2')
        volume = kg.kernel_volume
        shape = (in_channels, out_channels) if volume == 1 else (volume, in_channels, out_channels)
        self.kernel = nn.Parameter(torch.empty(shape))
        self.bias = nn.Parameter(torch.empty(1, out_channels)) if bias else None
        self._packed = None
        self._packed_tag = None
        self.reset_parameters()

    def _derived(self):
        tag = (self.kernel._version, self.kernel.data_ptr(), None if self.bias is None else self.bias._version)
        if self._packed_tag != tag:
            k = self.kernel.detach()
            b = None if self.bias is None else self.bias.detach().view(-1)
            d = {'w': k, 'b': b}
            if self.GENERATIVE and _packed_gen_ok(self.in_channels, self.out_channels):
                w_all = k.permute(1, 0, 2).reshape(self.in_channels, 8 * self.out_channels).contiguous()
                d['gen_w'] = [w_all] if w_all.shape[1] <= 128 else [w_all[:, :128].contiguous(), w_all[:, 128:].contiguous()]
                b_all = None if b is None else b.repeat(8)
                d['gen_b'] = [b_all] if (b_all is None or b_all.numel() <= 128) else [b_all[:128].contiguous(), b_all[128:].contiguous()]
            if not (self.GENERATIVE or self.TRANSPOSED) and self.ks == 3 and _split_k3_ok(self.in_channels, 0, self.out_channels):
                wt = torch.zeros((self.in_channels, 32), dtype=k.dtype, device=k.device)
                wt[:, :27] = k[:, :, 0].t()
                d['k3_w'] = wt
            self._packed, self._packed_tag = d, tag
        return self._packed

    def _padded_weights(self, c1: int, c2: int, plan):
        d = self._derived()
        key = ('pad', c1, c2) + tuple(plan)
        if key not in d:
            c1p, c2p, cop = plan
            k = self.kernel.detach()
            k = k.reshape(-1, k.shape[-2], k.shape[-1])
            w = torch.zeros((k.shape[0], c1p + c2p, cop), dtype=k.dtype, device=k.device)
            w[:, :c1, :self.out_channels] = k[:, :c1]
            if c2:
                w[:, c1p:c1p + c2, :self.out_channels] = k[:, c1:]
            b = None
            if self.bias is not None:
                b = torch.zeros(cop, dtype=k.dtype, device=k.device)
                b[:self.out_channels] = self.bias.detach().view(-1)
            d[key] = (w, b)
        return d[key]

    @staticmethod
    def _pad_cols(x: Optional[torch.Tensor], width: int) -> Optional[torch.Tensor]:
        if x is None or x.shape[1] == width:
            return x
        return torch.nn.functional.pad(x, (0, width - x.shape[1]))

    def _resolve(self, cm, src: _Map, coordinates):
        if self.GENERATIVE:
            return 'gen', cm._generated(src), None
        if self.TRANSPOSED:
            if coordinates is None:
                raise ValueError('a transposed convolution needs the target coordinate key')
            dst = cm._map(coordinates)
            if dst.parent is not src:
                raise ValueError('target map is not a stride-2 child of the input map')
            return ('gen', dst, None) if dst.generated else ('k2s2T', dst, dst.child_row)
        if self.ks == 1:
            return 'k1', src, None
        if self.ks == 3:
            if coordinates is not None and cm._map(coordinates) is not src:
                raise NotImplementedError('stride-1 convolution onto a different coordinate map')
            return 'k3', src, None
        dst = cm._ensure_parent(src)
        if src.generated:
            raise NotImplementedError('stride-2 convolution of a generated set')
        return 'k2s2', dst, src.child_row

    def _forward_autograd(self, x: SparseTensor, cm, src: _Map, coordinates, act: _Act, clip: float) -> SparseTensor:
        from .autograd import ConvSpec, sparse_conv
        feats = x.F
        kind, dst, table = self._resolve(cm, src, coordinates)
        tables = (cm._nbr27(src), cm._row_order(src, training=True)) if kind == 'k3' else () if table is None else (table,)
        spec = ConvSpec(kind, src.n, dst.n, *tables)
        if _fusable_in_training(act):
            from .autograd import sparse_conv_act
            out = sparse_conv_act(feats, self.kernel, self.bias, act.param if act.kind == ops.ACT_PRELU else None, spec, act.kind)
            out = _finish_autograd(out, None, _Act(), clip)
        else:
            out = _finish_autograd(sparse_conv(feats, self.kernel, spec), self.bias, act, clip)
        return SparseTensor(out, coordinate_map_key=dst.key, coordinate_manager=cm)

    def reset_parameters(self):
        fan = (self.out_channels if (self.TRANSPOSED or self.GENERATIVE) else self.in_channels) * \
            self.kernel_generator.kernel_volume
        bound = 1.0 / math.sqrt(fan)
        with torch.no_grad():
            self.kernel.uniform_(-bound, bound)
            if self.bias is not None:
                self.bias.uniform_(-bound, bound)

    def forward(self, x: SparseTensor, coordinates: Optional[CoordinateMapKey] = None, *, act: Optional[_Act] = None,
                clip: float = 0.0) -> SparseTensor:
        act = act or _Act()
        cm = x.coordinate_manager
        src = cm._map(x.coordinate_map_key)
        if torch.is_grad_enabled() and (self.kernel.requires_grad or any(p.requires_grad for p in x.parts)):
            return self._forward_autograd(x, cm, src, coordinates, act, clip)
        plan_rows = src.n
        if cm.independent_clouds and self.ks in (1, 3) and not (self.TRANSPOSED or self.GENERATIVE):
            c1, c2 = x.parts[0].shape[1], (x.parts[1].shape[1] if len(x.parts) > 1 else 0)
            edges = cm.batch_offsets(src)
            padded = [_pad_plan(c1, c2, self.out_channels, b - a) is not None for a, b in zip(edges[:-1], edges[1:]) if b > a]
            if any(padded) and not all(padded):
                big = self._forward_fused(x, cm, src, coordinates, act, clip, PAD_MIN_ROWS).F
                small = self._forward_fused(x, cm, src, coordinates, act, clip, 0).F
                out = torch.empty_like(small)
                for a, b in zip(edges[:-1], edges[1:]):
                    if b > a:
                        out[a:b] = (big if _pad_plan(c1, c2, self.out_channels, b - a) is not None else small)[a:b]
                return SparseTensor(out, coordinate_map_key=src.key, coordinate_manager=cm)
            plan_rows = PAD_MIN_ROWS if any(padded) else 0
        return self._forward_fused(x, cm, src, coordinates, act, clip, plan_rows)

    def _conv_padded(self, x1, x2, plan, n_out: int, act: _Act, clip: float, **table) -> torch.Tensor:
        wp, bp = self._padded_weights(x1.shape[1], 0 if x2 is None else x2.shape[1], plan)
        out = ops.conv_f32(self._pad_cols(x1, plan[0]), wp, plan[2], n_out, x2=self._pad_cols(x2, plan[1]), bias=bp, act=act.kind,
                           slope=act.slope, clip=clip, pack=True, **table)[:, :self.out_channels]
        return out.contiguous() if self.out_channels < 8 else out

    def _forward_fused(self, x: SparseTensor, cm: CoordinateManager, src: _Map, coordinates: Optional[CoordinateMapKey], act: _Act,
                       clip: float, plan_rows: int) -> SparseTensor:
        parts = x.parts
        x1 = parts[0]
        x2 = parts[1] if len(parts) > 1 else None
        c1, c2, c_out = x1.shape[1], (0 if x2 is None else x2.shape[1]), self.out_channels
        d = self._derived()
        w = d['w']
        ep = dict(bias=d['b'], act=act.kind, slope=act.slope, clip=clip)
        kw = dict(x2=x2, pack=True, **ep)
        kind, dst, table = self._resolve(cm, src, coordinates)
        form, shape = _layer_form(kind, c1, c2, c_out, plan_rows)
        if kind == 'gen':
            if form == 'gen' and self.GENERATIVE:
                out = torch.empty((src.n, 8 * c_out), dtype=torch.float32, device=x1.device)
                for h, wh in enumerate(d['gen_w']):
                    cols = wh.shape[1]
                    bh = d['gen_b'][h] if d['gen_b'][0] is not None else None
                    ops.conv_f32(x1, wh, cols, src.n, bias=bh, act=act.kind, slope=act.slope, clip=clip,
                                 out=out[:, h * 128: h * 128 + cols], pack=True)
                out = out.view(8 * src.n, c_out)
            else:
                out = ops.conv_f32(x1, w, c_out, src.n, groups=8, **kw)
        elif kind == 'k2s2T':
            order = None
            if x2 is None and ops.conv_k2s2t_use_sparse(c1, c_out, dst.n):
                order, sparse_table = cm._k2t_order(dst)
            if order is not None:
                out = ops.conv_k2s2t(x1, w, c_out, order, sparse_table, **ep)
            else:
                out = ops.conv_f32(x1, w, c_out, src.n, groups=8, out_map=table, om_os=8, om_gs=1, out_rows=dst.n, **kw)
        elif kind == 'k1':
            out = self._conv_padded(x1, x2, shape, src.n, act, clip) if form == 'pad' else ops.conv_f32(x1, w, c_out, src.n, **kw)
        elif kind == 'k3':
            if form == 'split':
                y = ops.conv_f32(x1, d['k3_w'], 32, src.n, pack=True)
                if src.generated and src.nbr27 is None and src.n == 8 * src.parent.n:
                    out = ops.gather_sum_generated(y, cm._nbr27(src.parent, True), **ep)
                else:
                    out = ops.gather_sum(y, cm._nbr27(src), 27, src.n, 1, src.n, **ep)
            elif form == 'pad':
                ro = cm._row_order(src) if shape[0] + shape[1] > 16 else None
                out = self._conv_padded(x1, x2, shape, src.n, act, clip, **cm._k3_table(src, True, ro), row_order=ro)
            elif x2 is None and c1 == 1 and getattr(x, '_fpcc_all_ones', False) and 4 <= c_out <= 32 and c_out % 4 == 0 \
                    and ops.conv_order(1, 0, c_out) == 0 and cm._mask27(src) is not None:
                out = ops.conv_ones_k3(cm._mask27(src), w, c_out, **ep)
            else:
                mfma = bool(ops.conv_plan(c1, c2, c_out, 27, 1).matrix)
                ro = cm._row_order(src) if mfma and c1 + c2 > 16 else None
                out = ops.conv_f32(x1, w, c_out, src.n, **cm._k3_table(src, mfma, ro), row_order=ro, **kw)
        else:
            ro = None
            if c1 + c2 > 16 and ops.conv_plan(c1, c2, c_out, 8, 1).matrix:
                ro, table = cm._k2_order(src)
            out = ops.conv_f32(x1, w, c_out, dst.n, nbr=table, n_offsets=8, nbr_ks=1, nbr_os=8, row_order=ro, **kw)
        return SparseTensor(out, coordinate_map_key=dst.key, coordinate_manager=cm)


class MinkowskiConvolution(_ConvBase):
    pass


def _fusable_in_training(act: _Act) -> bool:
    if act.kind != ops.ACT_PRELU:
        return True
    if act.param is None:
        return False
    cached = getattr(act.param, '_fpcc_host_value', None)
    if cached is None or cached[0] != act.param._version:
        cached = (act.param._version, float(act.param.detach().reshape(-1)[0].item()))
        act.param._fpcc_host_value = cached
    return cached[1] > 0


def refresh_prelu_cache(model: nn.Module) -> None:
    ps = [m.module.weight for m in model.modules() if isinstance(m, MinkowskiPReLU) and m.module.weight.numel() == 1]
    if ps:
        for p, v in zip(ps, torch.cat([p.detach().reshape(1) for p in ps]).tolist()):
            p._fpcc_host_value = (p._version, v)


def _finish_autograd(out: torch.Tensor, bias: Optional[torch.Tensor], act: _Act, clip: float) -> torch.Tensor:
    if bias is not None:
        out = out + bias.view(1, -1)
    if act.kind == ops.ACT_PRELU:
        out = torch.nn.functional.prelu(out, act.param if act.param is not None else act.slope)
    elif act.kind == ops.ACT_RELU:
        out = torch.relu(out)
    if clip > 0:
        from .autograd import BoundFunction
        from .entropy_models import scalar_tensor
        out = BoundFunction.apply(out, scalar_tensor(float(clip), torch.float32, out.device).view(()))
    return out


class MinkowskiConvolutionTranspose(_ConvBase):
    TRANSPOSED = True


class MinkowskiGenerativeConvolutionTranspose(_ConvBase):
    GENERATIVE = True


class MinkowskiLinear(nn.Module):
    def __init__(self, in_features, out_features, bias=True):
        super().__init__()
        self.linear = nn.Linear(in_features, out_features, bias=bias)
        self._wt = None
        self._wt_version = None

    def _weight_t(self) -> torch.Tensor:
        w = self.linear.weight
        if self._wt is None or self._wt_version != (w._version, w.data_ptr()):
            self._wt = w.detach().t().contiguous()
            self._wt_version = (w._version, w.data_ptr())
        return self._wt

    def forward(self, x: SparseTensor, *, act: Optional[_Act] = None, clip: float = 0.0) -> SparseTensor:
        act = act or _Act()
        if torch.is_grad_enabled() and (self.linear.weight.requires_grad or any(p.requires_grad for p in x.parts)):
            from .autograd import ConvSpec, sparse_conv
            n = x.parts[0].shape[0]
            if _fusable_in_training(act):
                from .autograd import sparse_linear_act
                out = sparse_linear_act(x.F, self.linear.weight, self.linear.bias, act.param if act.kind == ops.ACT_PRELU else None, act.kind)
                out = _finish_autograd(out, None, _Act(), clip)
            else:
                out = _finish_autograd(sparse_conv(x.F, self.linear.weight.t(), ConvSpec('k1', n, n)), self.linear.bias, act, clip)
            return SparseTensor(out, coordinate_map_key=x.coordinate_map_key, coordinate_manager=x.coordinate_manager)
        parts = x.parts
        b = self.linear.bias
        out = ops.conv_f32(parts[0], self._weight_t(), self.linear.out_features, parts[0].shape[0],
                           x2=parts[1] if len(parts) > 1 else None, bias=None if b is None else b.detach(),
                           act=act.kind, slope=act.slope, clip=clip, pack=True)
        return SparseTensor(out, coordinate_map_key=x.coordinate_map_key, coordinate_manager=x.coordinate_manager)


class _Pointwise(nn.Module):
    MODULE = None

    def __init__(self, *args, **kwargs):
        super().__init__()
        self.module = self.MODULE(*args, **kwargs)

    def forward(self, x: SparseTensor) -> SparseTensor:
        return SparseTensor(self.module(x.F), coordinate_map_key=x.coordinate_map_key,
                            coordinate_manager=x.coordinate_manager)


class MinkowskiReLU(_Pointwise):
    MODULE = nn.ReLU


class MinkowskiPReLU(_Pointwise):
    MODULE = nn.PReLU


class MinkowskiLeakyReLU(_Pointwise):
    MODULE = nn.LeakyReLU


class MinkowskiSigmoid(_Pointwise):
    MODULE = nn.Sigmoid


class MinkowskiBatchNorm(nn.Module):

    def __init__(self, num_features, eps=1e-5, momentum=0.1, affine=True, track_running_stats=True):
        super().__init__()
        self.bn = nn.BatchNorm1d(num_features, eps=eps, momentum=momentum, affine=affine, track_running_stats=track_running_stats)

    def forward(self, x: SparseTensor) -> SparseTensor:
        return SparseTensor(self.bn(x.F), coordinate_map_key=x.coordinate_map_key, coordinate_manager=x.coordinate_manager)


class _StridedPool(nn.Module):
    def __init__(self, kernel_size, stride=1, dilation=1, kernel_generator=None, dimension=3, **_):
        super().__init__()
        ks, st = _as_stride(kernel_size)[0], _as_stride(stride)[0]
        if ks != st:
            raise NotImplementedError('pooling over non-overlapping cells only (kernel_size == stride), as the codecs use it')
        self.cell = st


class MinkowskiMaxPooling(_StridedPool):

    def forward(self, x: SparseTensor, coordinates: Optional[CoordinateMapKey] = None) -> SparseTensor:
        cm = x.coordinate_manager
        src = cm._map(x.coordinate_map_key)
        if coordinates is None:
            dst = src
            for _ in range(self.cell.bit_length() - 1):
                dst = cm._ensure_parent(dst)
        else:
            dst = cm._map(coordinates)
        if (1 << dst.level) != (1 << src.level) * self.cell:
            raise ValueError('the target map does not have the pooled tensor stride')
        rows = cm._ancestor_rows(src, dst)
        f = x.F
        out = torch.full((dst.n, f.shape[1]), float('-inf'), dtype=f.dtype, device=f.device)
        out.scatter_reduce_(0, rows.unsqueeze(1).expand(-1, f.shape[1]), f, reduce='amax', include_self=True)
        return SparseTensor(out, coordinate_map_key=dst.key, coordinate_manager=cm)


class MinkowskiPoolingTranspose(_StridedPool):

    def forward(self, x: SparseTensor, coordinates: CoordinateMapKey) -> SparseTensor:
        cm = x.coordinate_manager
# ... 22 lines not shown
```

fastpcc_amd/hipops.py:

```python
import collections
import ctypes as C
import functools
from typing import List, Optional, Sequence, Tuple

import torch

from . import _native

_vp, _i64, _i32, _f32 = C.c_void_p, C.c_int64, C.c_int, C.c_float

ACT_NONE, ACT_PRELU, ACT_RELU = 0, 1, 2

_SIGS = {
    'fpcc_morton3d_encode': (_i32, [_vp, _i64, _i64, _i32, _i32, _i32, _vp, _vp]),
    'fpcc_hilbert3d_encode': (_i32, [_vp, _i64, _i64, _i32, _i32, _i32, _i32, _vp, _vp]),
    'fpcc_keys_from_coords': (_i32, [_vp, _i64, _i32, _i32, _vp, _vp]),
    'fpcc_coords_from_keys': (_i32, [_vp, _i64, _i32, _i32, _vp, _vp, _vp]),
    'fpcc_sort_keys': (_i64, [_vp, _i64, _i32, _vp, _vp, _vp, _i64, _vp]),
    'fpcc_unique_keys': (_i64, [_vp, _i64, _vp, _vp, _vp, _vp, _i64, _vp]),
    'fpcc_coarsen': (_i64, [_vp, _i64, _vp, _vp, _vp, _vp, _vp, _i64, _vp]),
    'fpcc_octree_level': (_i64, [_vp, _i64, _i64, _i32, _vp, _vp, _vp, _vp, _i64, _vp, _vp, _i64, _vp]),
    'fpcc_level_histogram': (_i64, [_vp, _i64, _i32, _vp, _vp]),
    'fpcc_level_histogram_clouds': (_i64, [_vp, _i64, _i32, _i32, _i32, _vp, _vp]),
    'fpcc_refine': (_i64, [_vp, _i64, _vp, _vp, _vp, _vp, _vp, _vp, _i64, _vp]),
    'fpcc_nbr27_search': (_i32, [_vp, _i64, _i32, _vp, _vp]),
    'fpcc_nbr27_from_parent': (_i32, [_vp, _vp, _i64, _vp, _i64, _vp, _vp, _vp]),
    'fpcc_nbr27_from_parent_ex': (_i32, [_vp, _vp, _i64, _vp, _i64, _vp, _vp, _vp, _vp, _vp]),
    'fpcc_conv_row_keys_masks': (_i32, [_vp, _i64, _i32, _vp, _vp]),
    'fpcc_gather_table_rows_i32': (_i32, [_vp, _i32, _vp, _i64, _vp, _vp]),
    'fpcc_mask27_from_parent': (_i32, [_vp, _vp, _i64, _vp, _i64, _vp, _vp, _vp]),
    'fpcc_conv_ones_k3_f32': (_i32, [_vp, _i64, _vp, _vp, _i32, _i32, _vp, C.c_float, _vp, _i32, _vp]),
    'fpcc_conv_f32': (_i32, [_vp, _i32, _i32, _vp, _i32, _i32, _vp, _i32, _i64, _i64, _vp, _vp, _i32, _i32,
                             _vp, _i64, _i64, _vp, _i32, _i64, _i32, _vp, _f32, _vp, _vp, _i64, _vp]),
    'fpcc_conv_f32_pk': (_i32, [_vp, _i32, _i32, _vp, _i32, _i32, _vp, _i32, _i64, _i64, _vp, _vp, _vp, _i32, _i32,
                                _vp, _i64, _i64, _vp, _i32, _i64, _i32, _vp, _f32, _vp, _vp, _i64, _vp]),
    'fpcc_conv_set_tuning': (_i32, [_i32, _i32]),
    'fpcc_conv_fold64_launches': (_i64, []),
    'fpcc_conv_k2s2t_order': (_i32, [_vp, _vp, _i64, _i64, _i32, _vp, _vp, _vp]),
    'fpcc_conv_k2s2t_f32': (_i32, [_vp, _i32, _i32, _vp, _vp, _vp, _vp, _i32, _vp, _i32, _i64, _i32, _vp, _f32, _vp]),
    'fpcc_conv_k2s2t_use_sparse': (_i32, [_i32, _i32, _i64]),
    'fpcc_conv_k2s2t_sparse_launches': (_i64, []),
    'fpcc_conv_debug_stamps': (_i32, [_vp, _i64]),
    'fpcc_conv_i8_debug_stamps': (_i32, [_vp, _i64]),
    'fpcc_time_next_launch': (_i32, [_vp, _vp]),
    'fpcc_transpose_table_i32': (_i32, [_vp, _i32, _i64, _vp, _i32, _vp]),
    'fpcc_numerics_version': (_i32, []),
    'fpcc_conv_packed_floats': (_i64, [_i32, _i32, _i32, _i32, _i32]),
    'fpcc_conv_pack_weights_f32': (_i32, [_vp, _i64, _i32, _i32, _vp, _vp]),
    'fpcc_conv_f32_natural_matrix': (_i32, [_i32, _i32, _i32, _i32, _i32]),
    'fpcc_conv_packed_floats_nat': (_i64, [_i32, _i32, _i32, _i32, _i32]),
    'fpcc_conv_pack_weights_nat_f32': (_i32, [_vp, _i64, _i32, _i32, _vp, _vp]),
    'fpcc_conv_natural_launches': (_i64, []),
    'fpcc_conv_natural_use_matrix': (_i32, [_i64]),
    'fpcc_nn_dist2': (_i32, [_vp, _i64, _i32, _vp, _i64, _vp, _vp, _vp]),
    'fpcc_knn3d': (_i32, [_vp, _i64, _vp, _i64, _i32, _vp, _vp, _vp]),
    'fpcc_sum_i64': (_i32, [_vp, _i64, _vp, _vp]),
    'fpcc_knn_voxels': (_i32, [_vp, _i64, _i32, _vp, _i64, _i32, _i32, _vp, _vp, _vp]),
    'fpcc_pca_normals': (_i32, [_vp, _i64, _i32, _vp, _i64, _i32, _vp, _vp]),
    'fpcc_nn_plane_dist2': (_i32, [_vp, _i64, _i32, _vp, _vp, _i64, _vp, _vp, _vp, _vp]),
    'fpcc_transfer_normals_ws_bytes': (_i64, [_i64, _i64]),
    'fpcc_transfer_normals': (_i32, [_vp, _i64, _vp, _vp, _vp, _i64, _vp, _i32, _vp, _vp, _i64, _vp]),
    'fpcc_sum_max_f64': (_i32, [_vp, _i64, _vp, _vp, _i64, _vp]),
    'fpcc_recolor_ws_bytes': (_i64, [_i64]),
    'fpcc_recolor': (_i32, [_vp, _i64, _vp, _i64, _vp, _i32, _vp, _vp, _i64, _vp]),
    'fpcc_keys_member': (_i32, [_vp, _i64, _vp, _i64, _vp, _vp]),
    'fpcc_transpose_weights_f32': (_i32, [_vp, _i32, _i32, _i32, _i32, _vp, _vp]),
    'fpcc_conv_wgrad_ws_bytes': (_i64, [_i32, _i32, _i32, _i32, _i64]),
    'fpcc_conv_wgrad_f32': (_i32, [_vp, _i32, _i32, _vp, _i32, _i32, _vp, _i32, _i64, _i64, _vp, _i64, _i64, _i32, _i64, _vp, _vp,
                                   _i32, _vp, _i64, _vp]),
    'fpcc_conv_wgrad_matrix': (_i32, [_i32, _i32]),
    'fpcc_epilogue_bwd_ws_bytes': (_i64, [_i64, _i32]),
    'fpcc_epilogue_bwd_f32': (_i32, [_vp, _i32, _vp, _i32, _i64, _i32, _i32, _vp, _vp, _i32, _vp, _vp, _vp, _i64, _vp]),
    'fpcc_noisy_normal_ws_bytes': (_i64, [_i64]),
    'fpcc_noisy_normal_bits_f32': (_i32, [_vp, _vp, _i64, _f32, _f32, _f32, _vp, _vp, _vp, _vp, _i64, _vp]),
    'fpcc_deep_factorized_ws_bytes': (_i64, [_i64, _i32]),
    'fpcc_deep_factorized_bits_f32': (_i32, [_vp, _i64, _i32, _i32, _vp, _vp, _vp, _f32, _vp, _i32, _vp, _vp, _i64, _vp]),
    'fpcc_conv_tile_keys': (_i32, [_vp, _i32, _vp, _i64, _i32, _vp, _vp]),
    'fpcc_conv_regroup_rows': (_i32, [_vp, _vp, _i64, _i32, _vp, _vp]),
    'fpcc_conv_group_order': (_i32, [_vp, _i64, _vp, _vp]),
    'fpcc_conv_row_keys': (_i32, [_vp, _i32, _i64, _i64, _i64, _i32, _vp, _vp, _vp]),
    'fpcc_conv_f32_ws_bytes': (_i64, [_i32, _i32, _i32, _i32, _i32, _i64]),
    'fpcc_conv_f32_order': (_i32, [_i32, _i32, _i32]),
    'fpcc_conv_f32_order_ex': (_i32, [_i32, _i32, _i32, _i32, _i32, _i64]),
    'fpcc_conv_f32_plan': (_i32, [_i32, _i32, _i32, _i32, _i32, _vp]),
    'fpcc_gather_sum_f32': (_i32, [_vp, _i32, _vp, _i32, _i64, _i64, _i64, _vp, _i32, _vp, _f32, _vp, _vp]),
    'fpcc_gather_sum_generated_f32': (_i32, [_vp, _i32, _vp, _i64, _vp, _i32, _vp, _f32, _vp, _vp]),
    'fpcc_logit_to_prob16': (_i32, [_vp, _i64, _vp, _vp]),
    'fpcc_quantize_symbols': (_i32, [_vp, _i64, _f32, _vp, _vp]),
    'fpcc_child_mask': (_i32, [_vp, _i64, _vp, _vp]),
    'fpcc_topk_keep': (_i64, [_vp, _i64, _i64, _vp, _vp, _i64, _vp]),
    'fpcc_topk_keep_cells': (_i64, [_vp, _i64, _vp, _i64, _i64, _vp, _vp, _i64, _vp]),
    'fpcc_topk_keep_batch': (_i64, [_vp, _i64, _vp, _i32, _vp, _i64, _vp, _vp, _vp, _i64, _vp]),
    'fpcc_gather_rows_f32': (_i32, [_vp, _i32, _i32, _vp, _i64, _vp, _i32, _vp]),
    'fpcc_compact_coords': (_i64, [_vp, _i64, _vp, _i32, _i32, _vp, _vp, _vp, _vp, _i64, _vp]),
    'fpcc_int_init': (_i32, []),
    'fpcc_hash_insert_coords': (_i32, [_vp, _vp, _i64, _vp, _i64, _vp]),
    'fpcc_hash_lookup_coords': (_i32, [_vp, _vp, _i64, _vp, _i64, _vp, _vp, _vp, _vp]),
    'fpcc_hash_insert_coords_bxyz': (_i32, [_vp, _vp, _i64, _vp, _i64, _vp]),
    'fpcc_hash_lookup_coords_bxyz': (_i32, [_vp, _vp, _i64, _vp, _i64, _vp, _vp, _vp, _vp]),
    'fpcc_hash_insert_keys': (_i32, [_vp, _vp, _i64, _vp, _i64, _vp]),
    'fpcc_hash_lookup_keys': (_i32, [_vp, _vp, _i64, _vp, _i64, _vp, _vp]),
    'fpcc_conv_i8': (_i32, [_vp, _i32, _i32, _vp, _i32, _i64, _i64, _i32, _vp, _i32, _vp, _vp, _vp, _vp, _vp, _i32, _i32,
                            _vp, _i32, _i32, _i32, _i64, _vp, _vp, _i64, _vp]),
    'fpcc_conv_i8_res': (_i32, [_vp, _i32, _i32, _vp, _i32, _i64, _i64, _i32, _vp, _i32, _vp, _vp, _vp, _vp, _vp, _i32, _i32,
                                _vp, _i32, _i32, _i32, _i64, _vp, _vp, _i32, _vp, _vp, _i64, _vp]),
    'fpcc_conv_i8_ws_bytes': (_i64, [_i32, _i32, _i32, _i32, _i64]),
    'fpcc_epilogue_i32': (_i32, [_vp, _i32, _vp, _vp, _vp, _i32, _vp, _i32, _i32, _vp, _i32, _i32, _i64, _i32, _vp, _vp]),
    'fpcc_prelu_i32': (_i32, [_vp, _vp, _vp, _i64, _vp, _vp]),
    'fpcc_softmax_i32': (_i32, [_vp, _i64, _i32, _vp, _vp]),
    'fpcc_logits_to_cdf16': (_i32, [_vp, _i64, _i32, _i32, _vp, _vp]),
    'fpcc_logits_to_ranges': (_i32, [_vp, _i64, _i32, _i32, _vp, _vp, _vp, _vp]),
    'fpcc_rans_binary_decode_dev': (_i32, [_vp, _i64, _vp, _i64, _vp, _vp, _vp, _vp]),
    'fpcc_simple_dec_pop_dev': (_i32, [_vp, _vp, _i64, _vp, _i64, _i64, _vp, _i64, _vp, _vp]),
    'fpcc_device_count': (_i32, []),
    'fpcc_clock_probe': (_i32, [_vp, _i32, _vp]),
    'fpcc_mlp_chain_f32': (_i32, [_vp, _vp]),
    'fpcc_mlp_chain_set_form': (_i32, [_i32]),
    'fpcc_pointwise_head_f32': (_i32, [_vp, _i32, _i32, _vp, _vp, _i32, _i32, _vp, _i32, _vp, _vp, _i32, _vp, _f32, _vp, _i64, _vp]),
    'fpcc_conv_i8_also': (_i32, [_vp, _i32, _i32, _vp, _i32, _i64, _i64, _i32, _vp, _i32, _vp, _vp, _vp, _vp, _vp, _i32, _i32,
                                 _vp, _i32, _i32, _i32, _i64, _vp, _vp, _i32, _vp, _vp, _i32, _vp, _i64, _vp]),
    'fpcc_epilogue_i32_also': (_i32, [_vp, _i32, _vp, _vp, _vp, _i32, _vp, _i32, _i32, _vp, _i32, _i32, _i64, _i32, _vp, _vp, _i32, _vp]),
    'fpcc_fill_bits_i8': (_i32, [_vp, _i64, _i32, _vp, _vp, _i32, _vp, _i32, _i32, _i32, _vp]),
    'fpcc_int_level_trunk': (_i64, [_vp, _i64, _vp, _vp, _vp, _vp, _vp, _vp, _vp, _i32, _vp, _vp, _i64, _vp]),
    'fpcc_int_level_expand': (_i64, [_vp, _i64, _i64, _vp, _vp, _i32, _vp, _vp, _vp, _vp, _vp, _vp, _vp, _vp, _vp, _i64, _vp]),
    'fpcc_octree_children': (_i64, [_vp, _vp, _vp, _i64, _i64, _i32, _vp, _vp, _vp, _vp, _i64, _vp, _vp, _vp, _i64, _vp]),
    'fpcc_conv_bf16_supported': (_i32, [_i32, _i32, _i32, _i32]),
    'fpcc_conv_bf16_wide_supported': (_i32, [_i32, _i32, _i32, _i32]),
    'fpcc_cast_f32_bf16': (_i32, [_vp, _i64, _i64, _i32, _vp, _i64, _vp]),
    'fpcc_conv_pack_weights_bf16': (_i32, [_vp, _i64, _i32, _i32, _i32, _i32, _i32, _i32, _vp, _vp]),
    'fpcc_conv_bf16': (_i32, [_vp, _i32, _i32, _vp, _i32, _i64, _i64, _vp, _vp, _i32, _i32, _vp, _i64, _i64, _vp, _i32, _i64, _i32,
                              _vp, _f32, _vp, _vp, _i64, _vp]),
    'fpcc_conv_wgrad_bf16_ws_bytes': (_i64, [_i32, _i32, _i32, _i32, _i64]),
    'fpcc_conv_wgrad_bf16': (_i32, [_vp, _i32, _i32, _vp, _i32, _i32, _vp, _i32, _i64, _i64, _vp, _i64, _i64, _i32, _i64, _vp, _vp,
                                    _i32, _vp, _i64, _vp]),
}
HIP_SYMBOLS = tuple(_SIGS) + ('fpcc_last_error',)
_BLOCKING_ENTRY_POINTS = ('fpcc_hilbert3d_encode', 'fpcc_conv_debug_stamps', 'fpcc_conv_i8_debug_stamps', 'fpcc_int_init')

_lib = None


def lib():
    global _lib
    if _lib is None:
        L = _native.hip()
        blocking = _native.hip_blocking()
        for name, (res, args) in _SIGS.items():
            fn = getattr(L, name)
            if name in _BLOCKING_ENTRY_POINTS:
                fn = getattr(blocking, name)
                setattr(L, name, fn)
            fn.restype = res
            fn.argtypes = args
        L.fpcc_last_error.restype = C.c_char_p
        L.fpcc_last_error.argtypes = []
        _lib = L
    return _lib


class FpccError(RuntimeError):
    pass


def no_gc_pause(fn):
    @functools.wraps(fn)
    def wrapped(*args, **kwargs):
        _gc_hold()
        try:
            return fn(*args, **kwargs)
        finally:
            _gc_release()
    return wrapped


_gc_lock = __import__('threading').Lock()
_gc_depth = 0
_gc_was_enabled = False


def _gc_hold():
    import gc
    global _gc_depth, _gc_was_enabled
    with _gc_lock:
        if _gc_depth == 0:
            _gc_was_enabled = gc.isenabled()
            gc.disable()
        _gc_depth += 1


def _gc_release():
# ... 143 lines not shown
    out, acc = [], 0
    for t in range(levels, 0, -1):
        acc += h[t]
        out.append(1 + acc)
    return out[::-1]


def level_counts_clouds(keys: torch.Tensor, levels: int, cloud_shift: int, n_clouds: int) -> List[List[int]]:
    n = keys.shape[0]
    hist = torch.empty((n_clouds, levels + 2), dtype=torch.int32, device=keys.device)
    _ok(lib().fpcc_level_histogram_clouds(_dev(keys, torch.int64, 'keys'), n, levels, int(cloud_shift), int(n_clouds),
                                          hist.data_ptr(), _stream()))
    h = hist.tolist()
    if sum(row[levels + 1] for row in h) != n:
        raise ValueError(f'a key carries a cloud index outside the batch of {n_clouds}: either the batch column is wrong or a coordinate '
                         f'(after subtracting its cloud\'s minimum) needs more than {cloud_shift // 3} bits per axis -- the Morton code of a '
                         f'cloud is {cloud_shift} bits wide (resolutions up to {1 << (cloud_shift // 3)})')
    out = [[0] * n_clouds for _ in range(levels + 1)]
    for c, row in enumerate(h):
        if row[levels + 1] and row[levels + 1] != 1 + sum(row[:levels + 1]):
            raise ValueError(f'cloud {c}: the keys are not unique ({row[levels + 1]} keys, {1 + sum(row[:levels + 1])} distinct)')
        out[0][c] = row[levels + 1]
        acc = 0
        for t in range(levels, 0, -1):
            acc += row[t]
            out[t][c] = acc + (1 if row[levels + 1] else 0)
    return out


def refine(pkeys: torch.Tensor, mask: torch.Tensor):
    m = pkeys.shape[0]
    dev = pkeys.device
    if mask.dtype == torch.bool:
        mask = mask.view(torch.uint8)
    if mask.numel() != 8 * m:
        raise ValueError('mask must have 8 entries per parent')
    keys = torch.empty(8 * m, dtype=torch.int64, device=dev)
    parent_of = torch.empty(8 * m, dtype=torch.int32, device=dev)
    child_row = torch.empty((m, 8), dtype=torch.int32, device=dev)
    count = torch.empty(1, dtype=torch.int32, device=dev)
    L = lib()
    ws, need = _ws(lambda: L.fpcc_refine(None, m, None, None, None, None, None, None, 0, None), dev)
    _ok(L.fpcc_refine(_dev(pkeys, torch.int64, 'pkeys'), m, _dev(mask, torch.uint8, 'mask'), keys.data_ptr(),
                      parent_of.data_ptr(), child_row.data_ptr(), count.data_ptr(), ws.data_ptr(), need, _stream()))
    return keys, parent_of, child_row, count


def nbr27_search(keys: torch.Tensor, bits: int) -> torch.Tensor:
    n = keys.shape[0]
    nbr = torch.empty((27, n), dtype=torch.int32, device=keys.device)
    _ok(lib().fpcc_nbr27_search(_dev(keys, torch.int64, 'keys'), n, bits, nbr.data_ptr(), _stream()))
    return nbr


def nbr27_from_parent(keys: Optional[torch.Tensor], parent_of: Optional[torch.Tensor], parent_nbr: torch.Tensor,
                      child_row: Optional[torch.Tensor], n: Optional[int] = None) -> torch.Tensor:
    m = parent_nbr.shape[1]
    if keys is None:
        n = 8 * m if n is None else n
    else:
        n = keys.shape[0]
    nbr = torch.empty((27, n), dtype=torch.int32, device=parent_nbr.device)
    _ok(lib().fpcc_nbr27_from_parent(_dev(keys, torch.int64, 'keys', True), _dev(parent_of, torch.int32, 'parent_of', True),
                                     n, _dev(parent_nbr, torch.int32, 'parent_nbr'), m,
                                     _dev(child_row, torch.int32, 'child_row', True), nbr.data_ptr(), _stream()))
    return nbr


def nbr27_from_parent_ex(keys: Optional[torch.Tensor], parent_of: Optional[torch.Tensor], parent_nbr: torch.Tensor,
                         child_row: Optional[torch.Tensor], n: Optional[int] = None):
    m = parent_nbr.shape[1]
    n = (8 * m if n is None else n) if keys is None else keys.shape[0]
    dev = parent_nbr.device
    nbr = torch.empty((27, n), dtype=torch.int32, device=dev)
    rows = torch.empty((n, 32), dtype=torch.int32, device=dev)
    masks = torch.empty(n, dtype=torch.int32, device=dev)
    _ok(lib().fpcc_nbr27_from_parent_ex(_dev(keys, torch.int64, 'keys', True), _dev(parent_of, torch.int32, 'parent_of', True),
                                        n, _dev(parent_nbr, torch.int32, 'parent_nbr'), m,
                                        _dev(child_row, torch.int32, 'child_row', True), nbr.data_ptr(), rows.data_ptr(),
                                        masks.data_ptr(), _stream()))
    return nbr, rows, masks


def gather_table_rows(rows: torch.Tensor, order: torch.Tensor) -> torch.Tensor:
    n, ld = rows.shape
    out = torch.empty_like(rows)
    _ok(lib().fpcc_gather_table_rows_i32(_dev(rows, torch.int32, 'rows'), ld, _dev(order, torch.int32, 'order'), n, out.data_ptr(), _stream()))
    return out


def mask27_from_parent(keys: Optional[torch.Tensor], parent_of: Optional[torch.Tensor], parent_nbr: torch.Tensor,
                       child_row: Optional[torch.Tensor], n: Optional[int] = None) -> torch.Tensor:
    m = parent_nbr.shape[1]
    n = (8 * m if n is None else n) if keys is None else keys.shape[0]
    masks = torch.empty(n, dtype=torch.int32, device=parent_nbr.device)
    _ok(lib().fpcc_mask27_from_parent(_dev(keys, torch.int64, 'keys', True), _dev(parent_of, torch.int32, 'parent_of', True),
                                      n, _dev(parent_nbr, torch.int32, 'parent_nbr'), m,
                                      _dev(child_row, torch.int32, 'child_row', True), masks.data_ptr(), _stream()))
    return masks


def conv_ones_k3(masks: torch.Tensor, w: torch.Tensor, c_out: int, *, bias: Optional[torch.Tensor] = None, act: int = 0,
                 slope: Optional[torch.Tensor] = None, clip: float = 0.0) -> torch.Tensor:
    n = masks.shape[0]
    if w.numel() != 27 * c_out or not w.is_contiguous():
        raise ValueError('weights must be contiguous [27, 1, c_out]')
    out = torch.empty((n, c_out), dtype=torch.float32, device=masks.device)
    _ok(lib().fpcc_conv_ones_k3_f32(_dev(masks, torch.int32, 'masks'), n, _dev(w, torch.float32, 'w'),
                                    _dev(bias, torch.float32, 'bias', True), c_out, act, _dev(slope, torch.float32, 'slope', True),
                                    float(clip), out.data_ptr(), c_out, _stream()))
    return out



def _rows2d(t: torch.Tensor, name: str):
    if t.dim() != 2 or t.dtype != torch.float32 or not t.is_cuda or t.stride(1) != 1:
        raise TypeError(f'{name} must be a 2-D float32 GPU tensor with unit column stride')
    return t.data_ptr(), t.shape[1], (t.stride(0) if t.shape[0] > 1 else max(t.shape[1], t.stride(0)))


_PACKED: 'collections.OrderedDict' = collections.OrderedDict()
_PACKED_MAX = 1024


def packed_weights(w: torch.Tensor, c1: int, c2: int, c_out: int, n_offsets: int, groups: int, fresh: bool = False) -> Optional[torch.Tensor]:
    image = conv_plan(c1, c2, c_out, n_offsets, groups).packed
    if not image:
        return None
    pack_fn = lib().fpcc_conv_pack_weights_f32 if image == 1 else lib().fpcc_conv_pack_weights_nat_f32
    if fresh:
        out = torch.empty(w.numel(), dtype=torch.float32, device=w.device)
        _ok(pack_fn(w.data_ptr(), groups * n_offsets, c1 + c2, c_out, out.data_ptr(), _stream()))
        return out
    key = (w.data_ptr(), w.numel(), c1 + c2, c_out)
    ent = _PACKED.get(key)
    if ent is not None and ent[1] == w._version:
        _PACKED.move_to_end(key)
        return ent[2]
    out = torch.empty(w.numel(), dtype=torch.float32, device=w.device)
    _ok(pack_fn(w.data_ptr(), groups * n_offsets, c1 + c2, c_out, out.data_ptr(), _stream()))
    _PACKED[key] = (w, w._version, out)
    while len(_PACKED) > _PACKED_MAX:
        _PACKED.popitem(last=False)
    return out


KNOB_WAVE_ON, KNOB_WAVE_NBW, KNOB_WAVE_SB, KNOB_WAVE_DBG, KNOB_MFMA_TILE, KNOB_POINTWISE_ROWS = 0, 1, 2, 3, 5, 6
KNOB_GROUPED_FOLD_ROWS = 4
KNOB_GROUPED_OFF, KNOB_GROUPED_NBW, KNOB_WAVE22_ROWS = 7, 8, 9
KNOB_PERSIST = 12
KNOB_FOLD64 = 13
KNOB_K2S2T_SPARSE = 14
KNOB_NATURAL_MFMA = 15
KNOB_LDS_ROWS, KNOB_LDS_ROW_BLOCKS = 10, 11


def conv_fold64_launches() -> int:
    return int(lib().fpcc_conv_fold64_launches())


def conv_natural_launches() -> int:
    return int(lib().fpcc_conv_natural_launches())


def numerics_version() -> int:
    return lib().fpcc_numerics_version()


def clock_probe(out2: torch.Tensor, spin_us: int = 20) -> None:
    _ok(lib().fpcc_clock_probe(_dev(out2, torch.int64, 'out2'), int(spin_us), _stream()))


def transpose_table(table: torch.Tensor, ld: int = 32) -> torch.Tensor:
    k, n = table.shape
    out = torch.empty((n, ld), dtype=torch.int32, device=table.device)
    _ok(lib().fpcc_transpose_table_i32(_dev(table, torch.int32, 'table', n == 0), k, n, out.data_ptr(), ld, _stream()))
    return out


def conv_debug_stamps(buf: Optional[torch.Tensor]) -> None:
    if buf is None:
        _ok(lib().fpcc_conv_debug_stamps(None, 0))
    else:
        _ok(lib().fpcc_conv_debug_stamps(_dev(buf, torch.int64, 'buf'), buf.numel()))


def conv_i8_debug_stamps(buf: Optional[torch.Tensor]) -> None:
    if buf is None:
        _ok(lib().fpcc_conv_i8_debug_stamps(None, 0))
    else:
        _ok(lib().fpcc_conv_i8_debug_stamps(_dev(buf, torch.int64, 'buf'), buf.numel()))


def conv_set_tuning(which: int, value: int) -> int:
    before = _ok(lib().fpcc_conv_set_tuning(int(which), int(value)))
    conv_plan.cache_clear()
    return before


CONV_TRACE = None
TRACE_LOCK = __import__('threading').RLock()
CLOCK_HOOK = None
_EVENT_POOL: list = []
_trace_tls = __import__('threading').local()


def set_thread_trace(trace) -> None:
    global _n_thread_traces
    had = getattr(_trace_tls, 'trace', None) is not None
    _trace_tls.trace = trace
    with TRACE_LOCK:
        _n_thread_traces += (trace is not None) - had


_n_thread_traces = 0


def _untraced_launch(fn, call) -> None:
    if _n_thread_traces:
        with TRACE_LOCK:
            _ok(fn(*call))
    else:
        _ok(fn(*call))


def _current_trace():
    t = getattr(_trace_tls, 'trace', None)
    return t if t is not None else CONV_TRACE


def reserve_trace_events(n: int) -> None:
    while len(_EVENT_POOL) < n:
        ev = torch.cuda.Event(enable_timing=True)
        ev.record()
        _EVENT_POOL.append(ev)


def _trace_event():
    if _EVENT_POOL:
        return _EVENT_POOL.pop()
    ev = torch.cuda.Event(enable_timing=True)
    ev.record()
    return ev


def _traced_launch(trace: list, fn, call, info) -> None:
    with TRACE_LOCK:
        ev0, ev1 = _trace_event(), _trace_event()
        if CLOCK_HOOK is not None:
            ev0.record()
            CLOCK_HOOK(ev0, info.get('n_out', 0), info.get('n_offsets', 1))
            _ok(fn(*call))
            ev1.record()
        else:
            _ok(lib().fpcc_time_next_launch(ev0.cuda_event, ev1.cuda_event))
            try:
                _ok(fn(*call))
            except BaseException:
                lib().fpcc_time_next_launch(None, None)
                raise
        trace.append((ev0, ev1, info))


def _conv_out(out: Optional[torch.Tensor], out_rows: Optional[int], n_out: int, groups: int, c_out: int, om_os: int, device):
    if out is None:
        rows = out_rows if out_rows is not None else n_out * groups
        out = torch.empty((rows, c_out), dtype=torch.float32, device=device)
    po, co, ldo = _rows2d(out, 'out')
    if co != c_out:
        raise ValueError('output width mismatch')
    return out, po, ldo, om_os if om_os else groups


def conv_f32(x1: torch.Tensor, w: torch.Tensor, c_out: int, n_out: int, *, x2: Optional[torch.Tensor] = None,
             nbr: Optional[torch.Tensor] = None, n_offsets: int = 1, nbr_ks: int = 0, nbr_os: int = 1,
             bias: Optional[torch.Tensor] = None, groups: int = 1, out_map: Optional[torch.Tensor] = None,
             om_os: int = 0, om_gs: int = 1, out: Optional[torch.Tensor] = None, out_rows: Optional[int] = None,
             act: int = ACT_NONE, slope: Optional[torch.Tensor] = None, clip: float = 0.0,
             row_order: Optional[torch.Tensor] = None, pack: bool = False) -> torch.Tensor:
    p1, c1, ld1 = _rows2d(x1, 'x1')
    if x2 is not None:
        p2, c2, ld2 = _rows2d(x2, 'x2')
    else:
        p2, c2, ld2 = None, 0, 0
    if w.dtype != torch.float32 or not w.is_cuda or not w.is_contiguous() or \
            w.numel() != groups * n_offsets * (c1 + c2) * c_out:
        raise ValueError(f'weights must be contiguous fp32 [{groups},{n_offsets},{c1 + c2},{c_out}], got {tuple(w.shape)}')
    out, po, ldo, om_os = _conv_out(out, out_rows, n_out, groups, c_out, om_os, x1.device)
    ws, ws_bytes = None, 0
    wp = packed_weights(w, c1, c2, c_out, n_offsets, groups, fresh=(pack == 'fresh')) if pack else None
    if wp is None and n_out > 0:
        ws_bytes = conv_plan(c1, c2, c_out, n_offsets, groups).ws_bytes
        if ws_bytes:
            ws = torch.empty(ws_bytes // 4, dtype=torch.float32, device=x1.device)
    fn = lib().fpcc_conv_f32_pk
    call = (p1, c1, ld1, p2, c2, ld2, _dev(nbr, torch.int32, 'nbr', True), n_offsets, nbr_ks, nbr_os,
            w.data_ptr(), None if wp is None else wp.data_ptr(),
            _dev(bias, torch.float32, 'bias', True), c_out, groups,
            _dev(out_map, torch.int32, 'out_map', True), om_os, om_gs, po, ldo, n_out, act,
            _dev(slope, torch.float32, 'slope', True), float(clip),
            _dev(row_order, torch.int32, 'row_order', True),
            None if ws is None else ws.data_ptr(), ws_bytes, _stream())
    trace = _current_trace()
    if trace is None:
        _untraced_launch(fn, call)
        return out
    plan = conv_plan(c1, c2, c_out, n_offsets, groups)
    on_matrix = plan.order != 0 or (plan.packed == 2 and conv_natural_uses_matrix(n_out * groups))
    _traced_launch(trace, fn, call, {'mfma': on_matrix, 'c_in': c1 + c2, 'c_out': c_out,
                                     'n_out': n_out, 'groups': groups, 'n_offsets': n_offsets, 'nbr': nbr,
                                     'nbr_ks': nbr_ks, 'nbr_os': nbr_os})
    return out


def conv_k2s2t_sparse_launches() -> int:
    return int(lib().fpcc_conv_k2s2t_sparse_launches())


def conv_k2s2t_use_sparse(c_in: int, c_out: int, n_children: int) -> bool:
    return bool(lib().fpcc_conv_k2s2t_use_sparse(int(c_in), int(c_out), int(n_children)))


K2S2T_WINDOW_LOG2 = 13


def conv_k2s2t_order(parent_of: torch.Tensor, child_row: torch.Tensor, n_children: int, window_log2: int = K2S2T_WINDOW_LOG2):
    dev = child_row.device
    order = torch.empty(n_children, dtype=torch.int32, device=dev)
    table = torch.empty((n_children, 8), dtype=torch.int32, device=dev)
    if parent_of.numel() < n_children or child_row.dim() != 2 or child_row.shape[1] != 8 or not child_row.is_contiguous():
        raise ValueError('parent_of [n_children] and a contiguous child_row [parents, 8] are needed')
    _ok(lib().fpcc_conv_k2s2t_order(_dev(parent_of, torch.int32, 'parent_of', n_children == 0), _dev(child_row, torch.int32, 'child_row', True),
                                    n_children, child_row.shape[0], window_log2, order.data_ptr(), table.data_ptr(), _stream()))
    return order, table


def conv_k2s2t(x: torch.Tensor, w: torch.Tensor, c_out: int, order: torch.Tensor, table: torch.Tensor, *,
               bias: Optional[torch.Tensor] = None, act: int = ACT_NONE, slope: Optional[torch.Tensor] = None,
               clip: float = 0.0) -> torch.Tensor:
    px, c_in, ld = _rows2d(x, 'x')
    n = order.numel()
    if w.dtype != torch.float32 or not w.is_cuda or not w.is_contiguous() or w.numel() != 8 * c_in * c_out:
        raise ValueError(f'weights must be contiguous fp32 [8,{c_in},{c_out}], got {tuple(w.shape)}')
    if table.shape != (n, 8) or not table.is_contiguous():
        raise ValueError('table must be the contiguous [n_children, 8] table of conv_k2s2t_order')
    wp = packed_weights(w, c_in, 0, c_out, 1, 8)
    if wp is None:
        raise ValueError(f'conv_k2s2t: no MFMA wave-kernel shape ({c_in} -> {c_out})')
    out = torch.empty((n, c_out), dtype=torch.float32, device=x.device)
    fn = lib().fpcc_conv_k2s2t_f32
    call = (px, c_in, ld, _dev(table, torch.int32, 'table', n == 0), _dev(order, torch.int32, 'order', n == 0), wp.data_ptr(),
            _dev(bias, torch.float32, 'bias', True), c_out, out.data_ptr(), c_out, n, act, _dev(slope, torch.float32, 'slope', True),
            float(clip), _stream())
    trace = _current_trace()
    if trace is None:
        _untraced_launch(fn, call)
        return out
    _traced_launch(trace, fn, call, {'mfma': True, 'c_in': c_in, 'c_out': c_out, 'n_out': n, 'groups': 1, 'n_offsets': 8, 'nbr': table,
                                     'nbr_ks': 1, 'nbr_os': 8, 'flops': 2.0 * n * c_in * c_out})
    return out


class _MlpLayer(C.Structure):
    _fields_ = [('w', _vp), ('w_packed', _vp), ('bias', _vp), ('slope', _vp), ('c_out', _i32), ('act', _i32), ('clip', _f32)]


class _MlpChain(C.Structure):
    _fields_ = [('x', _vp), ('cx', _i32), ('ldx', _i32), ('y', _vp), ('cy', _i32), ('ldy', _i32), ('cat_layer', _i32),
                ('n_layers', _i32), ('layers', _MlpLayer * 4), ('out', _vp), ('ldo', _i32), ('n', _i64)]


def pointwise_head_ok(c0: int, c1: int) -> bool:
    return (c0, c1) in ((16, 8), (8, 4))


def pointwise_head(x: torch.Tensor, w1: torch.Tensor, b1: Optional[torch.Tensor], act1: int, slope1: Optional[torch.Tensor], order1: int,
                   w2: torch.Tensor, b2: Optional[torch.Tensor], act2: int = ACT_NONE, slope2: Optional[torch.Tensor] = None,
                   clip: float = 0.0) -> torch.Tensor:
    px, c0, ldx = _rows2d(x, 'x')
    n = x.shape[0]
    if w1.dtype != torch.float32 or not w1.is_contiguous() or w1.shape[0] != c0 or w2.numel() != w1.shape[1] or not w2.is_contiguous():
        raise ValueError('weights must be contiguous fp32 [c0, c1] and [c1, 1]')
    out = torch.empty((n, 1), dtype=torch.float32, device=x.device)
    fn = lib().fpcc_pointwise_head_f32
    call = (px, c0, ldx, _dev(w1, torch.float32, 'w1'), _dev(b1, torch.float32, 'b1', True), w1.shape[1], int(act1),
            _dev(slope1, torch.float32, 'slope1', True), int(order1), _dev(w2, torch.float32, 'w2'),
            _dev(b2, torch.float32, 'b2', True), int(act2), _dev(slope2, torch.float32, 'slope2', True),
            float(clip), out.data_ptr(), n, _stream())
    trace = _current_trace()
    if trace is None:
        _untraced_launch(fn, call)
        return out
    _traced_launch(trace, fn, call, {'mfma': False, 'c_in': c0, 'c_out': 1, 'n_out': n, 'groups': 1, 'n_offsets': 1, 'nbr': None,
                                     'nbr_ks': 0, 'nbr_os': 1})
    return out


def mlp_chain_set_form(form: int) -> int:
    return lib().fpcc_mlp_chain_set_form(int(form))


def mlp_chain_ok(cx: int, widths, cat_layer: int = -1, cy: int = 0) -> bool:
    if not 1 <= len(widths) <= 4 or any(c not in (32, 64, 128) for c in widths):
        return False
    if not (cx == 1 or (cx % 32 == 0 and 32 <= cx <= 256)):
        return False
    if cat_layer == -1:
        return True
    return 1 <= cat_layer < len(widths) and cy % 32 == 0 and 32 <= cy <= 128


def mlp_chain(x: torch.Tensor, layers, y: Optional[torch.Tensor] = None, cat_layer: int = -1,
              out: Optional[torch.Tensor] = None) -> torch.Tensor:
    px, cx, ldx = _rows2d(x, 'x')
    n = x.shape[0]
    d = _MlpChain()
    d.x, d.cx, d.ldx, d.n, d.n_layers, d.cat_layer = px, cx, ldx, n, len(layers), cat_layer
    if y is not None:
        d.y, d.cy, d.ldy = _rows2d(y, 'y')
        if y.shape[0] != n:
            raise ValueError('concatenated operand has a different number of rows')
    keep = []
    c_in = cx
    flops = 0
    for l, (w, bias, act, slope, clip) in enumerate(layers):
        if l == cat_layer:
            c_in += d.cy
        if w.dtype != torch.float32 or not w.is_cuda or not w.is_contiguous() or w.dim() != 2 or w.shape[0] != c_in:
            raise ValueError(f'layer {l}: weights must be contiguous fp32 [{c_in}, c_out], got {tuple(w.shape)}')
        c_out = w.shape[1]
        L = d.layers[l]
        L.w = w.data_ptr()
        if c_in != 1:
            wp = packed_weights(w, c_in, 0, c_out, 1, 1)
            if wp is None:
                raise ValueError(f'layer {l}: {c_in} -> {c_out} has no packed form')
            keep.append(wp)
            L.w_packed = wp.data_ptr()
        L.bias = _dev(bias, torch.float32, 'bias', True)
        L.slope = _dev(slope, torch.float32, 'slope', True)
        L.c_out, L.act, L.clip = c_out, int(act), float(clip)
        flops += 2 * n * c_in * c_out
        c_in = c_out
    if out is None:
        out = torch.empty((n, c_in), dtype=torch.float32, device=x.device)
    d.out, co, d.ldo = _rows2d(out, 'out')
    if co != c_in or out.shape[0] != n:
        raise ValueError('output shape mismatch')
    fn, ref, stream = lib().fpcc_mlp_chain_f32, C.byref(d), _stream()
    trace = _current_trace()
    if trace is None:
        _untraced_launch(fn, (ref, stream))
        return out
    _traced_launch(trace, fn, (ref, stream), {'mfma': True, 'chain': True, 'c_in': cx, 'c_out': c_in, 'n_out': n, 'groups': 1, 'n_offsets': 1,
                                              'nbr': None, 'nbr_ks': 0, 'nbr_os': 1, 'flops': float(flops),
                                              'bytes': 4.0 * n * (cx + (d.cy if y is not None else 0) + c_in) + 4.0 * sum(w.numel() for w, *_ in layers),
                                              'layers': [tuple(w.shape) for w, *_ in layers]})
    return out


def nn_dist2(keys: torch.Tensor, bits: int, query: torch.Tensor, want_rows: bool = False):
    n = query.shape[0]
    d = torch.empty(n, dtype=torch.int64, device=query.device)
    rows = torch.empty(n, dtype=torch.int32, device=query.device) if want_rows else None
# ... 785 lines not shown
```

include/fpcc_hip.h:

```cpp
#ifndef FPCC_HIP_H_
#define FPCC_HIP_H_
#include <stdint.h>
#ifdef __cplusplus
extern "C" {
#endif

typedef enum {
    FPCC_OK = 0,
    FPCC_E_ARG = -1,
    FPCC_E_HIP = -2,
    FPCC_E_WORKSPACE = -3
} fpcc_status;

const char *fpcc_last_error(void);
int fpcc_device_count(void);
int fpcc_clock_probe(int64_t *out2, int spin_us, void *stream);


int fpcc_morton3d_encode(const int32_t *coords, int64_t n, int64_t row_stride, int col_bit0, int col_bit1, int col_bit2,
                         int64_t *keys_out, void *stream);

int fpcc_hilbert3d_encode(const int32_t *coords, int64_t n, int64_t row_stride, int col_x, int col_y, int col_z, int bits,
                          int64_t *keys_out, void *stream);

int fpcc_keys_from_coords(const int32_t *coords, int64_t n, int level, int bits, int64_t *keys_out, void *stream);
int fpcc_coords_from_keys(const int64_t *keys, int64_t n, int level, int bits, const int32_t *offset_xyz,
                          int32_t *coords_out, void *stream);

int64_t fpcc_sort_keys(const int64_t *keys_in, int64_t n, int end_bit, int64_t *keys_out, int32_t *perm_out,
                       void *ws, int64_t ws_bytes, void *stream);

int64_t fpcc_unique_keys(const int64_t *keys, int64_t n, int64_t *ukeys_out, int32_t *first_out, int32_t *count_out,
                         void *ws, int64_t ws_bytes, void *stream);

int64_t fpcc_coarsen(const int64_t *keys, int64_t n, int32_t *parent_of, int64_t *pkeys, int32_t *child_row,
                     int32_t *count_out, void *ws, int64_t ws_bytes, void *stream);
int64_t fpcc_octree_level(const int64_t *keys, int64_t n, int64_t m, int batch_shift, int64_t *pkeys, int32_t *coords, int32_t *bits,
                          int32_t *table, int64_t table_rows, int16_t *symbols, void *ws, int64_t ws_bytes, void *stream);
int64_t fpcc_level_histogram(const int64_t *keys, int64_t n, int levels, int32_t *hist, void *stream);
int64_t fpcc_level_histogram_clouds(const int64_t *keys, int64_t n, int levels, int cloud_shift, int n_clouds, int32_t *hist,
                                    void *stream);

int64_t fpcc_refine(const int64_t *pkeys, int64_t m, const uint8_t *mask, int64_t *keys_out, int32_t *parent_of,
                    int32_t *child_row, int32_t *count_out, void *ws, int64_t ws_bytes, void *stream);

int fpcc_nbr27_search(const int64_t *keys, int64_t n, int bits, int32_t *nbr, void *stream);
int fpcc_nbr27_from_parent(const int64_t *keys, const int32_t *parent_of, int64_t n, const int32_t *parent_nbr,
                           int64_t m, const int32_t *child_row, int32_t *nbr, void *stream);
int fpcc_nbr27_from_parent_ex(const int64_t *keys, const int32_t *parent_of, int64_t n, const int32_t *parent_nbr, int64_t m,
                              const int32_t *child_row, int32_t *nbr, int32_t *rows_out, uint32_t *masks_out, void *stream);
int fpcc_mask27_from_parent(const int64_t *keys, const int32_t *parent_of, int64_t n, const int32_t *parent_nbr, int64_t m,
                            const int32_t *child_row, uint32_t *masks_out, void *stream);

enum { FPCC_ACT_NONE = 0, FPCC_ACT_PRELU = 1, FPCC_ACT_RELU = 2 };

#define FPCC_NUMERICS_VERSION 3
#define FPCC_PAD_MIN_ROWS 8192
int fpcc_numerics_version(void);

int fpcc_conv_f32(const float *x1, int c1, int ld1, const float *x2, int c2, int ld2,
                  const int32_t *nbr, int n_offsets, int64_t nbr_ks, int64_t nbr_os,
                  const float *w, const float *bias, int c_out, int groups,
                  const int32_t *out_map, int64_t om_os, int64_t om_gs, float *out, int ldo, int64_t n_out,
                  int act, const float *slope, float clip, const int32_t *row_order, void *ws, int64_t ws_bytes,
                  void *stream);
int64_t fpcc_conv_packed_floats(int c1, int c2, int c_out, int n_offsets, int groups);
int fpcc_conv_f32_natural_matrix(int c1, int c2, int c_out, int n_offsets, int groups);
int64_t fpcc_conv_packed_floats_nat(int c1, int c2, int c_out, int n_offsets, int groups);
int fpcc_conv_pack_weights_nat_f32(const float *w, int64_t n_mats, int c_in, int c_out, float *w_packed, void *stream);
int fpcc_conv_natural_use_matrix(int64_t rows);
long long fpcc_conv_natural_launches(void);
int fpcc_conv_set_tuning(int which, int value);
long long fpcc_conv_fold64_launches(void);
int fpcc_conv_k2s2t_order(const int32_t *parent_of, const int32_t *child_row, int64_t n_children, int64_t n_parents, int window_log2,
                          int32_t *order_out, int32_t *table_out, void *stream);
int fpcc_conv_k2s2t_f32(const float *x, int c_in, int ld, const int32_t *table, const int32_t *order, const float *w_packed,
                        const float *bias, int c_out, float *out, int ldo, int64_t n_children, int act, const float *slope, float clip,
                        void *stream);
int fpcc_conv_k2s2t_use_sparse(int c_in, int c_out, int64_t n_children);
long long fpcc_conv_k2s2t_sparse_launches(void);
int fpcc_conv_debug_stamps(unsigned long long *buf, int64_t n_u64);
int fpcc_time_next_launch(void *start_event, void *end_event);
int fpcc_conv_i8_debug_stamps(unsigned long long *buf, int64_t n_u64);

int fpcc_conv_ones_k3_f32(const uint32_t *masks, int64_t n, const float *w, const float *bias, int c_out, int act,
                          const float *slope, float clip, float *out, int ldo, void *stream);
int fpcc_conv_pack_weights_f32(const float *w, int64_t n_mats, int c_in, int c_out, float *w_packed, void *stream);
int fpcc_conv_f32_pk(const float *x1, int c1, int ld1, const float *x2, int c2, int ld2,
                     const int32_t *nbr, int n_offsets, int64_t nbr_ks, int64_t nbr_os,
                     const float *w, const float *w_packed, const float *bias, int c_out, int groups,
                     const int32_t *out_map, int64_t om_os, int64_t om_gs, float *out, int ldo, int64_t n_out,
                     int act, const float *slope, float clip, const int32_t *row_order, void *ws, int64_t ws_bytes,
                     void *stream);
#define FPCC_MLP_CHAIN_MAX_LAYERS 4
typedef struct {
    const float *w;
    const float *w_packed;
    const float *bias;
    const float *slope;
    int c_out;
    int act;
    float clip;
} fpcc_mlp_layer;
typedef struct {
    const float *x; int cx; int ldx;
    const float *y; int cy; int ldy;
    int cat_layer;
    int n_layers;
    fpcc_mlp_layer layers[FPCC_MLP_CHAIN_MAX_LAYERS];
    float *out; int ldo;
    int64_t n;
} fpcc_mlp_chain;
int fpcc_mlp_chain_f32(const fpcc_mlp_chain *chain, void *stream);
int fpcc_mlp_chain_set_form(int form);
int fpcc_pointwise_head_f32(const float *x, int c0, int ldx, const float *w1, const float *b1, int c1, int act1,
                            const float *slope1, int order1, const float *w2, const float *b2, int act2, const float *slope2,
                            float clip, float *out, int64_t n, void *stream);
int fpcc_conv_row_keys(const int32_t *nbr, int n_offsets, int64_t nbr_ks, int64_t nbr_os, int64_t n, int window_log2,
                       int64_t *keys_out, uint32_t *masks_out, void *stream);
int fpcc_conv_row_keys_masks(const uint32_t *masks, int64_t n, int window_log2, int64_t *keys_out, void *stream);
int fpcc_gather_table_rows_i32(const int32_t *rows, int ld, const int32_t *order, int64_t n, int32_t *out, void *stream);
int fpcc_conv_tile_keys(const uint32_t *row_masks, int n_offsets, const int32_t *row_order, int64_t n, int group,
                        int64_t *keys_out, void *stream);
int fpcc_conv_group_order(const int64_t *group_keys, int64_t n_groups, int32_t *perm_out, void *stream);
int fpcc_conv_regroup_rows(const int32_t *row_order, const int32_t *group_perm, int64_t n, int group, int32_t *row_order_out,
                           void *stream);
typedef struct fpcc_conv_plan {
    int32_t order;
    int32_t matrix;
    int32_t packed;
    int32_t chunk;
    int64_t packed_floats;
    int64_t ws_bytes;
} fpcc_conv_plan;
int fpcc_conv_f32_plan(int c1, int c2, int c_out, int n_offsets, int groups, fpcc_conv_plan *plan);
int64_t fpcc_conv_f32_ws_bytes(int c1, int c2, int c_out, int n_offsets, int groups, int64_t n_out);
int fpcc_conv_f32_order(int c1, int c2, int c_out);
int fpcc_conv_f32_order_ex(int c1, int c2, int c_out, int n_offsets, int groups, int64_t n_out);

int64_t fpcc_conv_wgrad_ws_bytes(int c_in, int c_out, int n_offsets, int groups, int64_t n);
int fpcc_conv_wgrad_f32(const float *x, int c_in, int ldx, const float *dy, int c_out, int ldy,
                        const int32_t *nbr, int n_offsets, int64_t nbr_ks, int64_t nbr_os,
                        const int32_t *out_map, int64_t om_os, int64_t om_gs, int groups, int64_t n,
                        const int32_t *row_order, float *dw, int accumulate, void *ws, int64_t ws_bytes, void *stream);
int fpcc_conv_wgrad_matrix(int c_in, int c_out);
int fpcc_transpose_weights_f32(const float *w, int n_offsets, int c_in, int c_out, int flip, float *wt, void *stream);

int64_t fpcc_epilogue_bwd_ws_bytes(int64_t n, int c);
int fpcc_epilogue_bwd_f32(const float *y, int ldy, const float *dy, int lddy, int64_t n, int c, int act, const float *slope,
                          float *g, int ldg, float *dbias, float *dslope, void *ws, int64_t ws_bytes, void *stream);

int fpcc_gather_sum_f32(const float *y, int ldy, const int32_t *nbr, int n_offsets, int64_t nbr_ks, int64_t nbr_os,
                        int64_t n, const float *bias, int act, const float *slope, float clip, float *out, void *stream);
int fpcc_gather_sum_generated_f32(const float *y, int ldy, const int32_t *parent_nbr, int64_t m, const float *bias, int act,
                                  const float *slope, float clip, float *out, void *stream);

int fpcc_gather_rows_f32(const float *x, int c, int ld, const int32_t *index, int64_t n, float *out, int ldo, void *stream);
int fpcc_transpose_table_i32(const int32_t *table, int n_offsets, int64_t n, int32_t *rows_out, int ld, void *stream);


int fpcc_logit_to_prob16(const float *logit, int64_t n, uint16_t *prob_out, void *stream);

int fpcc_quantize_symbols(float *x, int64_t n, float scale, int32_t *symbols_out, void *stream);

int fpcc_child_mask(const int32_t *child_row, int64_t m, uint8_t *mask_out, void *stream);

int64_t fpcc_topk_keep(const float *logit, int64_t m, int64_t target, uint8_t *keep_out,
                       void *ws, int64_t ws_bytes, void *stream);

int64_t fpcc_compact_coords(const int64_t *pkeys, int64_t m, const uint8_t *mask, int level, int bits,
                            const int32_t *offset_xyz, int32_t *xyz_out, int32_t *count_out,
                            void *ws, int64_t ws_bytes, void *stream);

int64_t fpcc_topk_keep_cells(const float *logit, int64_t m, const int32_t *cell_of_group, int64_t n_cells, int64_t target,
                             uint8_t *keep_out, void *ws, int64_t ws_bytes, void *stream);

#define FPCC_TOPK_BATCH_MAX_SEGMENTS 256
int64_t fpcc_topk_keep_batch(const float *logit, int64_t m, const int64_t *seg_edges, int n_seg, const int32_t *cell_of_group,
                             int64_t n_cells, const int64_t *targets, uint8_t *keep_out, void *ws, int64_t ws_bytes, void *stream);

int64_t fpcc_deep_factorized_ws_bytes(int64_t n, int c);
int fpcc_deep_factorized_bits_f32(const float *y, int64_t n, int c, int ldy, const float *const *weights,
                                  const float *const *biases, const float *const *factors, float half_width,
                                  float *dy, int lddy, float *out, void *ws, int64_t ws_bytes, void *stream);

int64_t fpcc_noisy_normal_ws_bytes(int64_t n);
int fpcc_noisy_normal_bits_f32(const float *y, const float *index, int64_t n, float log_scale_offset, float log_scale_factor,
                               float half_width, float *dy, float *dindex, float *out, void *ws, int64_t ws_bytes, void *stream);

int fpcc_nn_dist2(const int64_t *keys, int64_t m, int bits, const int32_t *query, int64_t n, int64_t *dist2_out,
                  int32_t *nn_row_out, void *stream);
int fpcc_knn3d(const float *p1, int64_t n1, const float *p2, int64_t n2, int k, int64_t *idx_out, float *dist2_out, void *stream);
int fpcc_sum_i64(const int64_t *values, int64_t n, uint64_t *sum_out, void *stream);

int fpcc_knn_voxels(const int64_t *keys, int64_t m, int bits, const int32_t *query, int64_t n, int k, int start_level, int32_t *idx_out,
                    int64_t *dist2_out, void *stream);
int fpcc_pca_normals(const int64_t *keys, int64_t m, int bits, const int32_t *nbr, int64_t n, int k, double *normals_out, void *stream);
int fpcc_nn_plane_dist2(const int64_t *keys, int64_t m, int bits, const double *normals, const int32_t *query, int64_t n,
                        int64_t *dist2_out, int32_t *nn_row_out, double *plane_out, void *stream);
int64_t fpcc_transfer_normals_ws_bytes(int64_t n_a, int64_t n_b);
int fpcc_transfer_normals(const int64_t *keys_a, int64_t n_a, const int32_t *coords_a, const double *normals_a, const int64_t *keys_b,
                          int64_t n_b, const int32_t *coords_b, int bits, double *normals_b_out, void *ws, int64_t ws_bytes, void *stream);
int fpcc_sum_max_f64(const double *values, int64_t n, double *sum_max_out, void *ws, int64_t ws_bytes, void *stream);

int64_t fpcc_recolor_ws_bytes(int64_t m);
int fpcc_recolor(const int64_t *pred_keys, int64_t m, const int64_t *tgt_keys, int64_t n, const float *tgt_rgb, int bits,
                 float *rgb_out, void *ws, int64_t ws_bytes, void *stream);
int fpcc_keys_member(const int64_t *keys, int64_t m, const int64_t *query, int64_t n, int32_t *row_out, void *stream);


int fpcc_int_init(void);

int fpcc_hash_insert_coords(int64_t *table_keys, int32_t *table_vals, int64_t capacity, const int32_t *coords, int64_t n,
                            void *stream);
int fpcc_hash_lookup_coords(const int64_t *table_keys, const int32_t *table_vals, int64_t capacity, const int32_t *coords,
                            int64_t n, const int32_t *kernel_sizes_host, const int32_t *strides_host, int32_t *out,
                            void *stream);
int fpcc_hash_insert_coords_bxyz(int64_t *table_keys, int32_t *table_vals, int64_t capacity, const int32_t *coords, int64_t n,
                                 void *stream);
int fpcc_hash_lookup_coords_bxyz(const int64_t *table_keys, const int32_t *table_vals, int64_t capacity, const int32_t *coords,
                                 int64_t n, const int32_t *kernel_sizes_host, const int32_t *strides_host, int32_t *out,
                                 void *stream);
int fpcc_hash_insert_keys(int64_t *table_keys, int32_t *table_vals, int64_t capacity, const int64_t *keys, int64_t n,
                          void *stream);
int fpcc_hash_lookup_keys(const int64_t *table_keys, const int32_t *table_vals, int64_t capacity, const int64_t *keys,
// ... 89 lines not shown
```

Before: 92.60 Mpoints/s.

## Fuse network ends: ones-k3 into k2s2 conv, generative conv into classify head

Adds two fused kernels enabled by default through a new FPCC_FUSED_ENDS knob. At the encoder start, the k3 conv over all-ones occupancy masks is recomputed inside the following stride-2 MFMA conv instead of writing a 16-channel intermediate. At the decoder end, the last generative transpose conv (c_in to 8x16) is fused with the two-layer pointwise classify head when the head is the only reader. Both avoid materialising large per-child feature tensors in global memory. The cost is redundant recomputation of the 27-tap features per neighbour and more code paths to keep numerically consistent with the unfused ones.

```diff
diff --git a/fastpcc_amd/codecs/lossy_coord_v2/layers.py b/fastpcc_amd/codecs/lossy_coord_v2/layers.py
--- a/fastpcc_amd/codecs/lossy_coord_v2/layers.py
+++ b/fastpcc_amd/codecs/lossy_coord_v2/layers.py
@@ -17,15 +17,28 @@
     return mods[-1](x, clip=last_clip) if last_clip > 0 else mods[-1](x)
 
 
-def classify_head(seq: nn.Sequential, fea):
+def classify_head(seq: nn.Sequential, fea, sole_reader: bool = False):
     blocks = list(seq)
-    ok = len(blocks) == 2 and not torch.is_grad_enabled() and len(fea.parts) == 1
+    deferred = isinstance(fea, ME._DeferredTensor)
+    ok = len(blocks) == 2 and not torch.is_grad_enabled() and (deferred or len(fea.parts) == 1)
     if ok:
         a, b = blocks
         ok = all(isinstance(m, ConvBlock) and m.bn is None and m.conv.ks == 1 and
                  (m.act_module is None or isinstance(m.act_module, (ME.MinkowskiPReLU, ME.MinkowskiReLU))) for m in blocks) and \
             b.conv.out_channels == 1 and a.conv.out_channels == b.conv.in_channels and \
             ops.pointwise_head_ok(a.conv.in_channels, a.conv.out_channels)
+    gen = fea.take_recipe('gen_head') if ok and deferred and sole_reader and a.conv.in_channels == 16 else None
+    if gen is not None:
+        cm = fea.coordinate_manager
+        orders = {ME.summation_order('k1', a.conv.in_channels, 0, a.conv.out_channels, rows)
+                  for rows in cm.cloud_rows(cm._map(fea.coordinate_map_key)) if rows > 0}
+        if len(orders) == 1 and orders <= {0, 1}:
+            da, db = a.conv._derived(), b.conv._derived()
+            act1, act2 = ME._act_of(a.act_module), ME._act_of(b.act_module)
+            out = ops.gen_head(gen['x'], gen['w'], gen['b'], gen['act'].kind, gen['act'].slope, gen['clip'],
+                               da['w'].reshape(a.conv.in_channels, a.conv.out_channels), da['b'], act1.kind, act1.slope, orders.pop(),
+                               db['w'].reshape(-1), db['b'], act2.kind, act2.slope)
+            return ME.SparseTensor(out, coordinate_map_key=fea.coordinate_map_key, coordinate_manager=fea.coordinate_manager)
     x = fea.parts[0] if ok else None
     if not ok or x.dtype != torch.float32 or x.stride(1) != 1 or (x.shape[0] > 1 and x.stride(0) % 4) or x.data_ptr() % 16:
         return seq(fea)
@@ -157,7 +170,7 @@
         top = cm._map(fea.coordinate_map_key)
         for i, (up, classify) in enumerate(zip(self.upsample_blocks, self.classify_blocks)):
             fea = up(fea)
-            keep = self.get_keep(classify_head(classify, fea), points_num_list, top)
+            keep = self.get_keep(classify_head(classify, fea, sole_reader=(i == last)), points_num_list, top)
             if i != last:
                 fea = self.pruning(fea, keep)
             else:
diff --git a/fastpcc_amd/csrc/hip/conv.hip b/fastpcc_amd/csrc/hip/conv.hip
--- a/fastpcc_amd/csrc/hip/conv.hip
+++ b/fastpcc_amd/csrc/hip/conv.hip
@@ -989,16 +989,16 @@
 
 enum { kKnobWaveOn = 0, kKnobWaveNbw = 1, kKnobWaveSb = 2, kKnobStamps = 3, kKnobGroupedFoldRows = 4, kKnobMfmaCfg = 5, kKnobPointwiseRows = 6,
        kKnobGroupedOff = 7, kKnobGroupedNbw = 8, kKnobWave22Rows = 9, kKnobLdsRows = 10, kKnobLdsRowBlocks = 11, kKnobPersist = 12, kKnobFold64 = 13, kKnobK2s2tSparse = 14,
-       kKnobNaturalMfma = 15, kKnobCount = 16 };
-int g_knob[kKnobCount] = {-1, -1, -1, -1, -1, -1, -1, -1, -1, -1, -1, -1, -1, -1, -1, -1};
+       kKnobNaturalMfma = 15, kKnobFusedEnds = 16, kKnobCount = 17 };
+int g_knob[kKnobCount] = {-1, -1, -1, -1, -1, -1, -1, -1, -1, -1, -1, -1, -1, -1, -1, -1, -1};
 int knob(int k) {
     if (g_knob[k] < 0) {
         static const char *names[kKnobCount] = {"FPCC_CONV_WAVE", "FPCC_WAVE_NBW", "FPCC_WAVE_SB", "", "FPCC_GROUPED_FOLD_ROWS",
                                                 "FPCC_MFMA_TILE", "FPCC_POINTWISE_MIN_ROWS", "", "FPCC_GROUPED_NBW",
                                                 "FPCC_WAVE22_MIN_ROWS", "FPCC_LDS_MIN_ROWS", "FPCC_LDS_ROW_BLOCKS",
                                                 "FPCC_CONV_PERSIST", "FPCC_CONV_FOLD64", "FPCC_K2S2T_SPARSE",
-                                                "FPCC_CONV_NATURAL_MFMA"};
-        static const int defaults[kKnobCount] = {1, 0, 1, 0, 100 * 1024, 0, 32 * 1024, 0, 0, 0, 0, 2, 0, 0, 0, 2};
+                                                "FPCC_CONV_NATURAL_MFMA", "FPCC_FUSED_ENDS"};
+        static const int defaults[kKnobCount] = {1, 0, 1, 0, 100 * 1024, 0, 32 * 1024, 0, 0, 0, 0, 2, 0, 0, 0, 2, 1};
         const char *e = names[k][0] ? getenv(names[k]) : nullptr;
         g_knob[k] = e ? atoi(e) : defaults[k];
     }
@@ -1208,12 +1208,33 @@
     return nbw >= 2 ? launch_natural_cfg<2>(a, wp, s) : launch_natural_cfg<1>(a, wp, s);
 }
 
-template <int NBW, int NCH>
+struct HeadArgs {
+    const float *w1; const float *b1; int act1; const float *slope1; int order1;
+    const float *w2; const float *b2; int act2; const float *slope2; float clip; float *out;
+};
+constexpr int kHeadC0 = 16, kHeadC1 = 8;
+template <int NBW, int NCH, bool HEAD = false>
 __global__ __launch_bounds__(256, 2) void k_pointwise_wave(ConvArgs a, const float *__restrict__ wp, int nbt, unsigned n_row_blocks,
-                                                           unsigned waves_per_cg) {
+                                                           unsigned waves_per_cg, HeadArgs hd = HeadArgs{}) {
+    static_assert(kHeadC1 == 8 && (!HEAD || NBW == 4), "the head reads whole rows of 8 x 16 columns");
     constexpr int AC = NCH < 4 ? NCH : 4;
     constexpr int TW = 32 * NBW + 4;
-    __shared__ float s_tile[4][32 * TW];
+    __shared__ __attribute__((aligned(16))) float s_tile[4][32 * TW];
+    __shared__ __attribute__((aligned(16))) float s_hw1[HEAD ? kHeadC0 * kHeadC1 : 4];
+    __shared__ float s_hb1[HEAD ? kHeadC1 : 1], s_hw2[HEAD ? kHeadC1 : 1];
+    float sl1 = 0.0f, sl2 = 0.0f, b2 = 0.0f;
+    if constexpr (HEAD) {
+        for (int e = threadIdx.x; e < kHeadC0 * kHeadC1; e += 256) {
+            const int pos = e / kHeadC1, j = e - pos * kHeadC1;
+            const int c = hd.order1 ? (pos & ~7) + ((pos & 1) ? 4 : 0) + ((pos & 7) >> 1) : pos;
+            s_hw1[e] = hd.w1[c * kHeadC1 + j];
+        }
+        if (threadIdx.x < kHeadC1) { s_hb1[threadIdx.x] = hd.b1 ? hd.b1[threadIdx.x] : 0.0f; s_hw2[threadIdx.x] = hd.w2[threadIdx.x]; }
+        __syncthreads();
+        sl1 = (hd.act1 == FPCC_ACT_PRELU && hd.slope1) ? hd.slope1[0] : 0.0f;
+        sl2 = (hd.act2 == FPCC_ACT_PRELU && hd.slope2) ? hd.slope2[0] : 0.0f;
+        b2 = hd.b2 ? hd.b2[0] : 0.0f;
+    }
     const int lane = threadIdx.x & 63, wv = threadIdx.x >> 6;
     const int li = lane & 31, lh = lane >> 5;
     const unsigned n_cg = (unsigned)(nbt / NBW);
@@ -1300,6 +1321,35 @@
             for (int nb = 0; nb < NBW; ++nb) tile[r * TW + 32 * nb + li] = finish(acc[nb][reg], bias[nb], a.act, slope, a.clip);
         }
         __builtin_amdgcn_wave_barrier();
+        if constexpr (HEAD) {
+            const float *xr = tile + (lane >> 3) * TW + kHeadC0 * (lane & 7);
+            float h[4][kHeadC1];
+#pragma unroll
+            for (int q = 0; q < 4; ++q)
+#pragma unroll
+                for (int j = 0; j < kHeadC1; ++j) h[q][j] = 0.0f;
+#pragma unroll 2
+            for (int pos = 0; pos < kHeadC0; ++pos) {
+                const int c = hd.order1 ? (pos & ~7) + ((pos & 1) ? 4 : 0) + ((pos & 7) >> 1) : pos;
+                const f32x4 wa = *reinterpret_cast<const f32x4 *>(s_hw1 + pos * kHeadC1);
+                const f32x4 wb = *reinterpret_cast<const f32x4 *>(s_hw1 + pos * kHeadC1 + 4);
+#pragma unroll
+                for (int q = 0; q < 4; ++q) {
+                    const float xc = xr[8 * q * TW + c];
+                    h[q][0] = fmaf(xc, wa.x, h[q][0]); h[q][1] = fmaf(xc, wa.y, h[q][1]); h[q][2] = fmaf(xc, wa.z, h[q][2]); h[q][3] = fmaf(xc, wa.w, h[q][3]);
+                    h[q][4] = fmaf(xc, wb.x, h[q][4]); h[q][5] = fmaf(xc, wb.y, h[q][5]); h[q][6] = fmaf(xc, wb.z, h[q][6]); h[q][7] = fmaf(xc, wb.w, h[q][7]);
+                }
+            }
+#pragma unroll
+            for (int q = 0; q < 4; ++q) {
+                float lg = 0.0f;
+#pragma unroll
+                for (int j = 0; j < kHeadC1; ++j) lg = fmaf(finish(h[q][j], s_hb1[j], hd.act1, sl1, 0.0f), s_hw2[j], lg);
+                if (row0 + 8 * q + (lane >> 3) < a.n_out) hd.out[row0 * 8 + 64 * q + lane] = finish(lg, b2, hd.act2, sl2, hd.clip);
+            }
+            __builtin_amdgcn_wave_barrier();
+            continue;
+        }
         constexpr int LPR = 8 * NBW;
         constexpr int RPI = 64 / LPR;
         const int qr = lane / LPR, qc = lane % LPR;
@@ -1325,6 +1375,17 @@
     const unsigned waves = waves_per_cg * n_cg;
     hipLaunchKernelGGL((k_pointwise_wave<NBW, NCH>), dim3((waves + 3) / 4), dim3(256), 0, s, a, wp, nbt, row_blocks, waves_per_cg);
     return check_hip(hipGetLastError(), "k_pointwise_wave");
+}
+
+std::atomic<long long> g_fused_tail_launches{0};
+template <int NCH>
+int launch_gen_head_cfg(const ConvArgs &a, const float *wp, const HeadArgs &hd, hipStream_t s) {
+    const unsigned row_blocks = (unsigned)((a.n_out + 31) / 32);
+    unsigned waves = 256u * 4u * 2u;
+    if (waves > row_blocks) waves = row_blocks;
+    hipLaunchKernelGGL((k_pointwise_wave<4, NCH, true>), dim3((waves + 3) / 4), dim3(256), 0, s, a, wp, 4, row_blocks, waves, hd);
+    g_fused_tail_launches.fetch_add(1, std::memory_order_relaxed);
+    return check_hip(hipGetLastError(), "k_pointwise_wave(head)");
 }
 
 int launch_pointwise(const ConvArgs &a, const float *wp, hipStream_t s) {
@@ -1409,6 +1470,193 @@
                    float *out, int ldo, hipStream_t s) {
     hipLaunchKernelGGL((k_conv_ones_k3<CO, 1>), dim3(blocks_for(n, 256)), dim3(256), 0, s, masks, n, w, bias, act, slope, clip, out, ldo);
     return check_hip(hipGetLastError(), "k_conv_ones_k3");
+}
+
+struct OnesArgs {
+    const uint32_t *masks; const float *w1; const float *b1; int act1; const float *slope1; float clip1;
+};
+constexpr uint32_t kChildPresent = 0x80000000u;
+
+__device__ __forceinline__ float mask_bit(uint32_t m, int k) {
+    return __int_as_float((((int32_t)(m << (31 - k))) >> 31) & 0x3f800000);
+}
+
+template <int NBT, int WM, int WN>
+__global__ __launch_bounds__(64 * WM * WN, 3) void k_conv_k2s2_ones(ConvArgs a, OnesArgs f) {
+    constexpr int CH = 16;
+    using C = MfmaCfg<NBT, CH, WM, WN>;
+    constexpr int C_OUT = C::C_OUT;
+    constexpr int TM = C::TM;
+    constexpr int NBW = C::NBW;
+    constexpr int K2 = 8;
+
+    __shared__ __attribute__((aligned(16))) float sW[2 * CH * C_OUT];
+    __shared__ __attribute__((aligned(16))) float s_w1[27 * CH];
+    __shared__ __attribute__((aligned(16))) float s_b1[CH];
+    __shared__ int32_t s_nbr[K2 * TM];
+    __shared__ int32_t s_row[TM];
+    __shared__ unsigned s_mask[WM];
+
+    const int tid = threadIdx.x;
+    const int lane = tid & 63, wave = tid >> 6;
+    const int wr = wave % WM, wc = wave / WM;
+    const int li = lane & 31, lh = lane >> 5;
+    const unsigned tile = a.row_order ? blockIdx.x : xcd_remap(blockIdx.x, gridDim.x);
+    const int64_t row0 = (int64_t)tile * TM;
+
+    for (int e = tid; e < 27 * CH; e += C::THREADS) s_w1[e] = f.w1[e];
+    if (tid < CH) s_b1[tid] = f.b1 ? f.b1[tid] : 0.0f;
+    for (int r = tid; r < TM; r += C::THREADS)
+        s_row[r] = row0 + r < a.n_out ? (a.row_order ? a.row_order[row0 + r] : (int32_t)(row0 + r)) : -1;
+    const bool by_pos = a.row_order && table_is_row_major(a);
+    for (int e = tid; e < K2 * TM; e += C::THREADS) {
+        const int k = e / TM, r = e % TM;
+        int32_t v = -1;
+        if (row0 + r < a.n_out) {
+            const int64_t row = a.row_order ? (int64_t)a.row_order[row0 + r] : row0 + r;
+            v = a.nbr[(int64_t)k * a.nbr_ks + (by_pos ? row0 + r : row) * a.nbr_os];
+        }
+        s_nbr[e] = v;
+    }
+    __syncthreads();
+    unsigned wmask = 0;
+    for (int k = 0; k < K2; ++k)
+        if (__ballot(s_nbr[k * TM + wr * 32 + li] >= 0) != 0ull) wmask |= 1u << k;
+    if (lane == 0 && wc == 0) s_mask[wr] = wmask;
+    __syncthreads();
+    unsigned tmask = 0;
+#pragma unroll
+    for (int i = 0; i < WM; ++i) tmask |= s_mask[i];
+    const int n_stages = __popc(tmask);
+
+    f32x16 acc[NBW];
+#pragma unroll
+    for (int nb = 0; nb < NBW; ++nb)
+#pragma unroll
+        for (int r = 0; r < 16; ++r) acc[nb][r] = 0.0f;
+
+    const int32_t *my_nbr = s_nbr + wr * 32;
+    const float slope1 = (f.act1 == FPCC_ACT_PRELU && f.slope1) ? f.slope1[0] : 0.0f;
+    const f32x4 b1lo = *reinterpret_cast<const f32x4 *>(s_b1 + 4 * lh), b1hi = *reinterpret_cast<const f32x4 *>(s_b1 + 8 + 4 * lh);
+    auto fetch_m = [&](int k) -> uint32_t {
+        const int32_t idx = my_nbr[k * TM + li];
+        const uint32_t m = f.masks[idx >= 0 ? idx : 0];
+        return idx >= 0 ? (m | kChildPresent) : 0u;
+    };
+    auto features = [&](uint32_t m, f32x4 (&ra)[2]) {
+        f32x4 lo = {0.0f, 0.0f, 0.0f, 0.0f}, hi = {0.0f, 0.0f, 0.0f, 0.0f};
+#pragma unroll 3
+        for (int k = 0; k < 27; ++k) {
+            const float bit = mask_bit(m, k);
+            const f32x4 wl = *reinterpret_cast<const f32x4 *>(s_w1 + k * CH + 4 * lh);
+            const f32x4 wh = *reinterpret_cast<const f32x4 *>(s_w1 + k * CH + 8 + 4 * lh);
+            lo.x = fmaf(bit, wl.x, lo.x); lo.y = fmaf(bit, wl.y, lo.y); lo.z = fmaf(bit, wl.z, lo.z); lo.w = fmaf(bit, wl.w, lo.w);
+            hi.x = fmaf(bit, wh.x, hi.x); hi.y = fmaf(bit, wh.y, hi.y); hi.z = fmaf(bit, wh.z, hi.z); hi.w = fmaf(bit, wh.w, hi.w);
+        }
+        const bool present = (m & kChildPresent) != 0u;
+        ra[0].x = present ? finish(lo.x, b1lo.x, f.act1, slope1, f.clip1) : 0.0f;
+        ra[0].y = present ? finish(lo.y, b1lo.y, f.act1, slope1, f.clip1) : 0.0f;
+        ra[0].z = present ? finish(lo.z, b1lo.z, f.act1, slope1, f.clip1) : 0.0f;
+        ra[0].w = present ? finish(lo.w, b1lo.w, f.act1, slope1, f.clip1) : 0.0f;
+        ra[1].x = present ? finish(hi.x, b1hi.x, f.act1, slope1, f.clip1) : 0.0f;
+        ra[1].y = present ? finish(hi.y, b1hi.y, f.act1, slope1, f.clip1) : 0.0f;
+        ra[1].z = present ? finish(hi.z, b1hi.z, f.act1, slope1, f.clip1) : 0.0f;
+        ra[1].w = present ? finish(hi.w, b1hi.w, f.act1, slope1, f.clip1) : 0.0f;
+    };
+
+    f32x4 ra[2], rw[C::W_PIECES];
+    if (n_stages > 0) {
+        unsigned rest = tmask;
+        int k_cur = __ffs(rest) - 1;
+        int k_next = k_cur;
+        uint32_t m_nxt = fetch_m(k_cur);
+        fetch_w<C, CH>(a.w, CH, tid, k_cur, 0, rw);
+        stash_w<C>(sW, tid, rw);
+        __syncthreads();
+        for (int s = 0; s < n_stages; ++s) {
+            rest &= rest - 1;
+            k_next = rest ? __ffs(rest) - 1 : k_cur;
+            const uint32_t m_cur = m_nxt;
+            m_nxt = fetch_m(k_next);
+            fetch_w<C, CH>(a.w, CH, tid, k_next, 0, rw);
+            if ((wmask >> k_cur) & 1u) {
+                features(m_cur, ra);
+                stage_compute<C, CH>(ra, sW + (s & 1) * CH * C_OUT, wc, li, lh, acc);
+            }
+            stash_w<C>(sW + ((s + 1) & 1) * CH * C_OUT, tid, rw);
+            __syncthreads();
+            k_cur = k_next;
+        }
+    }
+
+    const float slope = (a.act == FPCC_ACT_PRELU && a.slope) ? a.slope[0] : 0.0f;
+    float bias[NBW];
+#pragma unroll
+    for (int nb = 0; nb < NBW; ++nb) bias[nb] = a.bias ? a.bias[32 * (wc * NBW + nb) + li] : 0.0f;
+    int64_t dsts[16];
+#pragma unroll
+    for (int reg = 0; reg < 16; ++reg) dsts[reg] = s_row[wr * 32 + (reg & 3) + 8 * (reg >> 2) + 4 * lh];
+#pragma unroll
+    for (int reg = 0; reg < 16; ++reg) {
+        const int64_t dst = dsts[reg];
+        if (dst < 0) continue;
+#pragma unroll
+        for (int nb = 0; nb < NBW; ++nb)
+            a.out[dst * a.ldo + 32 * (wc * NBW + nb) + li] = finish(acc[nb][reg], bias[nb], a.act, slope, a.clip);
+    }
+}
+
+__global__ __launch_bounds__(256) void k_conv_k2s2_ones_valu(ConvArgs a, OnesArgs f) {
+    constexpr int JB = 16;
+    const int64_t o = (int64_t)blockIdx.x * 256 + threadIdx.x;
+    const int j0 = (int)blockIdx.y * JB;
+    if (o >= a.n_out) return;
+    const int c_in = a.c1;
+    float acc[JB];
+#pragma unroll
+    for (int j = 0; j < JB; ++j) acc[j] = 0.0f;
+    const float slope1 = (f.act1 == FPCC_ACT_PRELU && f.slope1) ? f.slope1[0] : 0.0f;
+#pragma unroll 1
+    for (int k = 0; k < a.n_off; ++k) {
+        const int32_t idx = a.nbr[(int64_t)k * a.nbr_ks + o * a.nbr_os];
+        if (idx < 0) continue;
+        const uint32_t m = f.masks[idx];
+        const float *wk = a.w + (int64_t)k * c_in * a.c_out + j0;
+#pragma unroll 1
+        for (int c = 0; c < c_in; ++c) {
+            float x = 0.0f;
+#pragma unroll 9
+            for (int kk = 0; kk < 27; ++kk) x = fmaf(mask_bit(m, kk), f.w1[kk * c_in + c], x);
+            x = finish(x, f.b1 ? f.b1[c] : 0.0f, f.act1, slope1, f.clip1);
+            const float *wr = wk + (int64_t)c * a.c_out;
+#pragma unroll
+            for (int j = 0; j < JB; ++j)
+                if (j0 + j < a.c_out) acc[j] = fmaf(x, wr[j], acc[j]);
+        }
+    }
+    const float slope = (a.act == FPCC_ACT_PRELU && a.slope) ? a.slope[0] : 0.0f;
+#pragma unroll
+    for (int j = 0; j < JB; ++j)
+        if (j0 + j < a.c_out) a.out[o * a.ldo + j0 + j] = finish(acc[j], a.bias ? a.bias[j0 + j] : 0.0f, a.act, slope, a.clip);
+}
+
+std::atomic<long long> g_fused_head_launches{0};
+
+template <int NBT, int WM, int WN>
+int launch_k2s2_ones_cfg(const ConvArgs &a, const OnesArgs &f, hipStream_t s) {
+    constexpr int TM = 32 * WM;
+    hipLaunchKernelGGL((k_conv_k2s2_ones<NBT, WM, WN>), dim3((unsigned)((a.n_out + TM - 1) / TM)), dim3(64 * WM * WN), 0, s, a, f);
+    return check_hip(hipGetLastError(), "k_conv_k2s2_ones");
+}
+
+template <int NBT>
+int launch_k2s2_ones(const ConvArgs &a, const OnesArgs &f, hipStream_t s) {
+    const int forced = knob(kKnobMfmaCfg) - 1;
+    constexpr int WNS = NBT >= 2 ? 2 : 1;
+    const int cfg = forced >= 0 ? forced : (NBT <= 2 && a.n_out >= 128 * 1024) ? 0 : a.n_out >= 32 * 1024 ? 1 : 2;
+    if (cfg == 0) return launch_k2s2_ones_cfg<NBT, 4, 1>(a, f, s);
+    if (cfg == 1) return launch_k2s2_ones_cfg<NBT, 2, WNS>(a, f, s);
+    return launch_k2s2_ones_cfg<NBT, 1, NBT>(a, f, s);
 }
 
 template <int JB>
@@ -1486,6 +1734,74 @@
     }
 }
 
+extern "C" int fpcc_conv_fused_ends(void) { return knob(kKnobFusedEnds) != 0 ? 1 : 0; }
+
+extern "C" long long fpcc_conv_fused_head_launches(void) { return g_fused_head_launches.load(std::memory_order_relaxed); }
+
+extern "C" int fpcc_conv_k2s2_ones_ok(int c_in, int c_out) {
+    if (c_in < 4 || c_in > 32 || c_in % 4 || c_out < 32 || c_out % 32) return 0;
+    const fpcc_conv_plan plan = conv_plan(c_in, 0, c_out, 8, 1);
+    return (plan.chunk == 16 || !plan.matrix) ? 1 : 0;
+}
+
+extern "C" int fpcc_conv_k2s2_ones_f32(const uint32_t *masks, int64_t n_children, const float *w1, const float *b1, int c_in, int act1,
+                                       const float *slope1, float clip1, const int32_t *child_row, int64_t nbr_ks, int64_t nbr_os,
+                                       const float *w, const float *bias, int c_out, float *out, int ldo, int64_t n_out, int act,
+                                       const float *slope, float clip, const int32_t *row_order, void *stream) {
+    LaunchBracket timed(stream);
+    if (n_out < 0 || n_children < 0 || ldo < c_out) return fail_arg("conv_k2s2_ones: sizes out of range");
+    if (!fpcc_conv_k2s2_ones_ok(c_in, c_out))
+        return fail_arg("conv_k2s2_ones: 4 <= c_in <= 32 and c_out multiples of 4 and 32, on the 16-channel matrix kernel or the VALU kernel");
+    if (n_out == 0) return FPCC_OK;
+    if (n_children == 0) return fail_arg("conv_k2s2_ones: parents without a child map");
+    if (!masks || !w1 || !child_row || !w || !out) return fail_arg("conv_k2s2_ones: null pointer");
+    if ((act != FPCC_ACT_NONE && act != FPCC_ACT_PRELU && act != FPCC_ACT_RELU) ||
+        (act1 != FPCC_ACT_NONE && act1 != FPCC_ACT_PRELU && act1 != FPCC_ACT_RELU))
+        return fail_arg("conv_k2s2_ones: unknown activation");
+    if ((act == FPCC_ACT_PRELU && !slope) || (act1 == FPCC_ACT_PRELU && !slope1)) return fail_arg("conv_k2s2_ones: PReLU needs a slope pointer");
+    ConvArgs a{nullptr, c_in, c_in, nullptr, 0, 0, child_row, 8, nbr_ks, nbr_os, w, bias, c_out, 1,
+               nullptr, 0, 0, out, ldo, n_out, act, slope, clip, row_order};
+    const OnesArgs f{masks, w1, b1, act1, slope1, clip1};
+    hipStream_t s = as_stream(stream);
+    const fpcc_conv_plan plan = conv_plan(c_in, 0, c_out, 8, 1);
+    g_fused_head_launches.fetch_add(1, std::memory_order_relaxed);
+    if (plan.chunk == 16) {
+        if (!aligned16(w)) return fail_arg("conv_k2s2_ones: the MFMA path needs 16-byte aligned weights");
+        if (c_out == 128) return launch_k2s2_ones<4>(a, f, s);
+        if (c_out == 64) return launch_k2s2_ones<2>(a, f, s);
+        return launch_k2s2_ones<1>(a, f, s);
+    }
+    if (row_order) return fail_arg("conv_k2s2_ones: row_order is a feature of the matrix path");
+    if ((c_out + 15) / 16 > 65535) return fail_arg("conv_k2s2_ones: too many output channels");
+    hipLaunchKernelGGL(k_conv_k2s2_ones_valu, dim3(blocks_for(n_out, 256), (c_out + 15) / 16), dim3(256), 0, s, a, f);
+    return check_hip(hipGetLastError(), "k_conv_k2s2_ones_valu");
+}
+
+extern "C" long long fpcc_conv_fused_tail_launches(void) { return g_fused_tail_launches.load(std::memory_order_relaxed); }
+
+extern "C" int fpcc_gen_head_ok(int c_in, int c_mid) { return ((c_in == 32 || c_in == 64) && c_mid == kHeadC0) ? 1 : 0; }
+
+extern "C" int fpcc_gen_head_f32(const float *x, int c_in, int ld, const float *w_packed, const float *bias, int act, const float *slope,
+                                 float clip, const float *w1, const float *b1, int act1, const float *slope1, int order1, const float *w2,
+                                 const float *b2, int act2, const float *slope2, float clip2, float *out, int64_t n_parents, void *stream) {
+    LaunchBracket timed(stream);
+    if (n_parents < 0 || (c_in != 32 && c_in != 64) || ld < c_in || ld % 4) return fail_arg("gen_head: c_in 32 or 64, row stride a multiple of 4");
+    if (order1 != 0 && order1 != 1) return fail_arg("gen_head: hidden-layer order must be 0 (natural) or 1 (MFMA chain)");
+    if (n_parents == 0) return FPCC_OK;
+    if (32 * ((n_parents + 31) / 32) > 0x7fffffffll) return fail_arg("gen_head: too many rows");
+    if (!x || !w_packed || !w1 || !w2 || !out || !aligned16(x) || !aligned16(w_packed)) return fail_arg("gen_head: null or unaligned pointer");
+    const int acts[3] = {act, act1, act2};
+    for (int v : acts)
+        if (v != FPCC_ACT_NONE && v != FPCC_ACT_PRELU && v != FPCC_ACT_RELU) return fail_arg("gen_head: unknown activation");
+    if ((act == FPCC_ACT_PRELU && !slope) || (act1 == FPCC_ACT_PRELU && !slope1) || (act2 == FPCC_ACT_PRELU && !slope2))
+        return fail_arg("gen_head: PReLU needs a slope pointer");
+    ConvArgs a{x, c_in, ld, nullptr, 0, 0, nullptr, 1, 0, 1, nullptr, bias, 8 * kHeadC0, 1,
+               nullptr, 0, 0, nullptr, 8 * kHeadC0, n_parents, act, slope, clip, nullptr};
+    const HeadArgs hd{w1, b1, act1, slope1, order1, w2, b2, act2, slope2, clip2, out};
+    hipStream_t s = as_stream(stream);
+    return c_in == 64 ? launch_gen_head_cfg<2>(a, w_packed, hd, s) : launch_gen_head_cfg<1>(a, w_packed, hd, s);
+}
+
 extern "C" int fpcc_conv_debug_stamps(unsigned long long *buf, int64_t n_u64) {
     if (n_u64 < 0 || (n_u64 > 0 && !buf)) return fail_arg("conv_debug_stamps: null buffer");
     const long long cap = buf ? n_u64 : 0;
diff --git a/fastpcc_amd/engine.py b/fastpcc_amd/engine.py
--- a/fastpcc_amd/engine.py
+++ b/fastpcc_amd/engine.py
@@ -539,6 +539,41 @@
         return f'SparseTensor(shape={tuple(self.shape)}, key={self.coordinate_map_key})'
 
 
+class _DeferredTensor(SparseTensor):
+
+    def __init__(self, make, recipe, shape, device, coordinate_map_key: CoordinateMapKey, coordinate_manager: CoordinateManager):
+        self.coordinate_manager, self.coordinate_map_key = coordinate_manager, coordinate_map_key
+        self._make, self._recipe, self._made = make, recipe, None
+        self._shape, self._device = torch.Size(shape), device
+
+    @property
+    def _parts(self):
+        if self._made is None:
+            self._made = (self._make(),)
+            self._make = self._recipe = None
+        return self._made
+
+    @_parts.setter
+    def _parts(self, parts):
+        self._made = parts
+
+    def take_recipe(self, kind: str):
+        r = self._recipe
+        return r[1] if self._made is None and r is not None and r[0] == kind else None
+
+    @property
+    def shape(self):
+        return self._shape
+
+    @property
+    def device(self):
+        return self._device
+
+    @property
+    def dtype(self):
+        return torch.float32
+
+
 def _average_duplicates(features, cm, key, coordinates, tensor_stride):
     m = cm._map(key)
     level = m.level
@@ -770,6 +805,9 @@
 
     def _forward_fused(self, x: SparseTensor, cm: CoordinateManager, src: _Map, coordinates: Optional[CoordinateMapKey], act: _Act,
                        clip: float, plan_rows: int) -> SparseTensor:
+        head = self._fused_head(x, cm, src, coordinates, act, clip)
+        if head is not None:
+            return head
         parts = x.parts
         x1 = parts[0]
         x2 = parts[1] if len(parts) > 1 else None
@@ -782,6 +820,12 @@
         form, shape = _layer_form(kind, c1, c2, c_out, plan_rows)
         if kind == 'gen':
             if form == 'gen' and self.GENERATIVE:
+                if x2 is None and len(d['gen_w']) == 1 and ops.gen_head_ok(c1, c_out) and ops.conv_fused_ends() and x1.stride(1) == 1 \
+                        and (src.n <= 1 or x1.stride(0) % 4 == 0) and x1.data_ptr() % 16 == 0:
+                    recipe = dict(x=x1, w=d['gen_w'][0], b=d['gen_b'][0], act=act, clip=clip)
+                    return _DeferredTensor(lambda: ops.conv_f32(x1, recipe['w'], 8 * c_out, src.n, bias=recipe['b'], act=act.kind,
+                                                                slope=act.slope, clip=clip, pack=True).view(8 * src.n, c_out),
+                                           ('gen_head', recipe), (8 * src.n, c_out), x1.device, dst.key, cm)
                 out = torch.empty((src.n, 8 * c_out), dtype=torch.float32, device=x1.device)
                 for h, wh in enumerate(d['gen_w']):
                     cols = wh.shape[1]
@@ -813,7 +857,11 @@
                 out = self._conv_padded(x1, x2, shape, src.n, act, clip, **cm._k3_table(src, True, ro), row_order=ro)
             elif x2 is None and c1 == 1 and getattr(x, '_fpcc_all_ones', False) and 4 <= c_out <= 32 and c_out % 4 == 0 \
                     and ops.conv_order(1, 0, c_out) == 0 and cm._mask27(src) is not None:
-                out = ops.conv_ones_k3(cm._mask27(src), w, c_out, **ep)
+                masks = cm._mask27(src)
+                if ops.conv_fused_ends():
+                    return _DeferredTensor(lambda: ops.conv_ones_k3(masks, w, c_out, **ep), ('ones_k3', dict(masks=masks, w=w, ep=ep)),
+                                           (src.n, c_out), masks.device, src.key, cm)
+                out = ops.conv_ones_k3(masks, w, c_out, **ep)
             else:
                 mfma = bool(ops.conv_plan(c1, c2, c_out, 27, 1).matrix)
                 ro = cm._row_order(src) if mfma and c1 + c2 > 16 else None
@@ -823,6 +871,26 @@
             if c1 + c2 > 16 and ops.conv_plan(c1, c2, c_out, 8, 1).matrix:
                 ro, table = cm._k2_order(src)
             out = ops.conv_f32(x1, w, c_out, dst.n, nbr=table, n_offsets=8, nbr_ks=1, nbr_os=8, row_order=ro, **kw)
+        return SparseTensor(out, coordinate_map_key=dst.key, coordinate_manager=cm)
+
+
+    def _fused_head(self, x: SparseTensor, cm, src: _Map, coordinates, act: _Act, clip: float) -> Optional[SparseTensor]:
+        if not isinstance(x, _DeferredTensor) or self.TRANSPOSED or self.GENERATIVE or (self.ks, self.st) != (2, 2):
+            return None
+        c1, c_out = x.shape[1], self.out_channels
+        if not ops.conv_k2s2_ones_ok(c1, c_out) or src.generated:
+            return None
+        first = x.take_recipe('ones_k3')
+        if first is None:
+            return None
+        d = self._derived()
+        dst = cm._ensure_parent(src)
+        ro, table = None, src.child_row
+        if c1 > 16 and ops.conv_plan(c1, 0, c_out, 8, 1).matrix:
+            ro, table = cm._k2_order(src)
+        fe = first['ep']
+        out = ops.conv_k2s2_ones(first['masks'], first['w'], c1, table, d['w'], c_out, dst.n, bias1=fe['bias'], act1=fe['act'],
+                                 slope1=fe['slope'], clip1=fe['clip'], bias=d['b'], act=act.kind, slope=act.slope, clip=clip, row_order=ro)
         return SparseTensor(out, coordinate_map_key=dst.key, coordinate_manager=cm)
 
 
diff --git a/fastpcc_amd/hipops.py b/fastpcc_amd/hipops.py
--- a/fastpcc_amd/hipops.py
+++ b/fastpcc_amd/hipops.py
@@ -36,6 +36,15 @@
                                 _vp, _i64, _i64, _vp, _i32, _i64, _i32, _vp, _f32, _vp, _vp, _i64, _vp]),
     'fpcc_conv_set_tuning': (_i32, [_i32, _i32]),
     'fpcc_conv_fold64_launches': (_i64, []),
+    'fpcc_conv_fused_ends': (_i32, []),
+    'fpcc_conv_k2s2_ones_ok': (_i32, [_i32, _i32]),
+    'fpcc_conv_k2s2_ones_f32': (_i32, [_vp, _i64, _vp, _vp, _i32, _i32, _vp, _f32, _vp, _i64, _i64, _vp, _vp, _i32, _vp, _i32, _i64, _i32,
+                                       _vp, _f32, _vp, _vp]),
+    'fpcc_conv_fused_head_launches': (_i64, []),
+    'fpcc_gen_head_ok': (_i32, [_i32, _i32]),
+    'fpcc_gen_head_f32': (_i32, [_vp, _i32, _i32, _vp, _vp, _i32, _vp, _f32, _vp, _vp, _i32, _vp, _i32, _vp, _vp, _i32, _vp, _f32, _vp,
+                                 _i64, _vp]),
+    'fpcc_conv_fused_tail_launches': (_i64, []),
     'fpcc_conv_k2s2t_order': (_i32, [_vp, _vp, _i64, _i64, _i32, _vp, _vp, _vp]),
     'fpcc_conv_k2s2t_f32': (_i32, [_vp, _i32, _i32, _vp, _vp, _vp, _vp, _i32, _vp, _i32, _i64, _i32, _vp, _f32, _vp]),
     'fpcc_conv_k2s2t_use_sparse': (_i32, [_i32, _i32, _i64]),
@@ -485,11 +494,24 @@
 KNOB_FOLD64 = 13
 KNOB_K2S2T_SPARSE = 14
 KNOB_NATURAL_MFMA = 15
+KNOB_FUSED_ENDS = 16
 KNOB_LDS_ROWS, KNOB_LDS_ROW_BLOCKS = 10, 11
 
 
 def conv_fold64_launches() -> int:
     return int(lib().fpcc_conv_fold64_launches())
+
+
+def conv_fused_ends() -> bool:
+    return bool(lib().fpcc_conv_fused_ends())
+
+
+def conv_fused_head_launches() -> int:
+    return int(lib().fpcc_conv_fused_head_launches())
+
+
+def conv_fused_tail_launches() -> int:
+    return int(lib().fpcc_conv_fused_tail_launches())
 
 
 def conv_natural_launches() -> int:
@@ -643,6 +665,63 @@
     _traced_launch(trace, fn, call, {'mfma': on_matrix, 'c_in': c1 + c2, 'c_out': c_out,
                                      'n_out': n_out, 'groups': groups, 'n_offsets': n_offsets, 'nbr': nbr,
                                      'nbr_ks': nbr_ks, 'nbr_os': nbr_os})
+    return out
+
+
+def conv_k2s2_ones_ok(c_in: int, c_out: int) -> bool:
+    return bool(lib().fpcc_conv_k2s2_ones_ok(int(c_in), int(c_out)))
+
+
+def conv_k2s2_ones(masks: torch.Tensor, w1: torch.Tensor, c_in: int, child_row: torch.Tensor, w: torch.Tensor, c_out: int, n_out: int, *,
+                   bias1: Optional[torch.Tensor] = None, act1: int = ACT_NONE, slope1: Optional[torch.Tensor] = None, clip1: float = 0.0,
+                   bias: Optional[torch.Tensor] = None, act: int = ACT_NONE, slope: Optional[torch.Tensor] = None, clip: float = 0.0,
+                   row_order: Optional[torch.Tensor] = None) -> torch.Tensor:
+    if w1.numel() != 27 * c_in or not w1.is_contiguous() or w.numel() != 8 * c_in * c_out or not w.is_contiguous():
+        raise ValueError('weights must be contiguous [27, 1, c_in] and [8, c_in, c_out]')
+    if child_row.dim() != 2 or child_row.shape[1] != 8 or child_row.shape[0] < n_out or not child_row.is_contiguous():
+        raise ValueError('child_row must be a contiguous [n_out, 8] table')
+    out = torch.empty((n_out, c_out), dtype=torch.float32, device=masks.device)
+    fn = lib().fpcc_conv_k2s2_ones_f32
+    call = (_dev(masks, torch.int32, 'masks', n_out == 0), masks.shape[0], _dev(w1, torch.float32, 'w1'), _dev(bias1, torch.float32, 'bias1', True),
+            int(c_in), int(act1), _dev(slope1, torch.float32, 'slope1', True), float(clip1), _dev(child_row, torch.int32, 'child_row', n_out == 0),
+            1, 8, _dev(w, torch.float32, 'w'), _dev(bias, torch.float32, 'bias', True), int(c_out), out.data_ptr(), c_out, int(n_out),
+            int(act), _dev(slope, torch.float32, 'slope', True), float(clip), _dev(row_order, torch.int32, 'row_order', True), _stream())
+    trace = _current_trace()
+    if trace is None:
+        _untraced_launch(fn, call)
+        return out
+    _traced_launch(trace, fn, call, {'mfma': conv_plan(c_in, 0, c_out, 8, 1).order != 0, 'c_in': c_in, 'c_out': c_out, 'n_out': n_out,
+                                     'groups': 1, 'n_offsets': 8, 'nbr': child_row, 'nbr_ks': 1, 'nbr_os': 8})
+    return out
+
+
+def gen_head_ok(c_in: int, c_mid: int) -> bool:
+    return bool(lib().fpcc_gen_head_ok(int(c_in), int(c_mid)))
+
+
+def gen_head(x: torch.Tensor, w_gen: torch.Tensor, bias: Optional[torch.Tensor], act: int, slope: Optional[torch.Tensor], clip: float,
+             w1: torch.Tensor, b1: Optional[torch.Tensor], act1: int, slope1: Optional[torch.Tensor], order1: int,
+             w2: torch.Tensor, b2: Optional[torch.Tensor], act2: int = ACT_NONE, slope2: Optional[torch.Tensor] = None,
+             clip2: float = 0.0) -> torch.Tensor:
+    px, c_in, ld = _rows2d(x, 'x')
+    n = x.shape[0]
+    if w_gen.dtype != torch.float32 or not w_gen.is_contiguous() or tuple(w_gen.shape) != (c_in, 128):
+        raise ValueError('generative weights must be contiguous fp32 [c_in, 8 * 16]')
+    if w1.dtype != torch.float32 or not w1.is_contiguous() or tuple(w1.shape) != (16, 8) or w2.numel() != 8 or not w2.is_contiguous():
+        raise ValueError('head weights must be contiguous fp32 [16, 8] and [8, 1]')
+    wp = packed_weights(w_gen, c_in, 0, 128, 1, 1)
+    out = torch.empty((8 * n, 1), dtype=torch.float32, device=x.device)
+    fn = lib().fpcc_gen_head_f32
+    call = (px, c_in, ld, wp.data_ptr(), _dev(bias, torch.float32, 'bias', True), int(act), _dev(slope, torch.float32, 'slope', True),
+            float(clip), _dev(w1, torch.float32, 'w1'), _dev(b1, torch.float32, 'b1', True), int(act1),
+            _dev(slope1, torch.float32, 'slope1', True), int(order1), _dev(w2, torch.float32, 'w2'), _dev(b2, torch.float32, 'b2', True),
+            int(act2), _dev(slope2, torch.float32, 'slope2', True), float(clip2), out.data_ptr(), n, _stream())
+    trace = _current_trace()
+    if trace is None:
+        _untraced_launch(fn, call)
+        return out
+    _traced_launch(trace, fn, call, {'mfma': True, 'c_in': c_in, 'c_out': 128, 'n_out': n, 'groups': 1, 'n_offsets': 1, 'nbr': None,
+                                     'nbr_ks': 0, 'nbr_os': 1})
     return out
 
 
diff --git a/include/fpcc_hip.h b/include/fpcc_hip.h
--- a/include/fpcc_hip.h
+++ b/include/fpcc_hip.h
@@ -71,6 +71,18 @@
 int fpcc_conv_natural_use_matrix(int64_t rows);
 long long fpcc_conv_natural_launches(void);
 int fpcc_conv_set_tuning(int which, int value);
+int fpcc_conv_fused_ends(void);
+int fpcc_conv_k2s2_ones_ok(int c_in, int c_out);
+int fpcc_conv_k2s2_ones_f32(const uint32_t *masks, int64_t n_children, const float *w1, const float *b1, int c_in, int act1,
+                            const float *slope1, float clip1, const int32_t *child_row, int64_t nbr_ks, int64_t nbr_os,
+                            const float *w, const float *bias, int c_out, float *out, int ldo, int64_t n_out, int act,
+                            const float *slope, float clip, const int32_t *row_order, void *stream);
+long long fpcc_conv_fused_head_launches(void);
+int fpcc_gen_head_ok(int c_in, int c_mid);
+int fpcc_gen_head_f32(const float *x, int c_in, int ld, const float *w_packed, const float *bias, int act, const float *slope, float clip,
+                      const float *w1, const float *b1, int act1, const float *slope1, int order1, const float *w2, const float *b2,
+                      int act2, const float *slope2, float clip2, float *out, int64_t n_parents, void *stream);
+long long fpcc_conv_fused_tail_launches(void);
 long long fpcc_conv_fold64_launches(void);
 int fpcc_conv_k2s2t_order(const int32_t *parent_of, const int32_t *child_row, int64_t n_children, int64_t n_parents, int window_log2,
                           int32_t *order_out, int32_t *table_out, void *stream);
```

Result: no change. 92.67 Mpoints/s, median of 3 (+0.1%).
